# Hfx-J/SGTD

Measured on AMD Instinct MI355X. Metric: query frames/sec vs map size (descriptor build + candidate selection), higher is better.
Workload: dtype f64

## Files before the change

include/sgtd_accel.h:

```cpp
#ifndef SGTD_ACCEL_H
#define SGTD_ACCEL_H

#include <stddef.h>
#include <stdint.h>

#ifdef __cplusplus
extern "C" {
#endif

typedef enum sgtd_status {
  SGTD_OK = 0,
  SGTD_ERR_INVALID = -1,
  SGTD_ERR_NO_DEVICE = -2,
  SGTD_ERR_HIP = -3,
  SGTD_ERR_CAPACITY = -4,
  SGTD_ERR_FRAME_LIMIT = -5,
  SGTD_ERR_UNSUPPORTED = -6,
  SGTD_ERR_STATE = -7,
  SGTD_ERR_IO = -8
} sgtd_status;

typedef struct sgtd_config {
  int32_t descriptor_near_num;
  int32_t candidate_num;
  int32_t max_frame_n;
  int32_t device_id;
  double descriptor_min_len;
  double descriptor_max_len;
  double std_side_resolution;
  double rough_dis_threshold;
  uint32_t first_frame_id;
  uint32_t reserved;
} sgtd_config;

typedef struct sgtd_desc_soa {
  double *side;
  double *angle;
  double *center;
  float *vertex;
  int32_t *label;
  uint32_t *frame;
  int32_t *node_id;
} sgtd_desc_soa;

typedef struct sgtd_stats {
  int64_t n_entries;
  int64_t n_buckets;
  int64_t n_frames;
  int64_t last_queries;
  int64_t last_D;
  int64_t last_P;
  int64_t last_M;
  int64_t last_cand_pairs;
  int64_t hbm_bytes_table;
  float ms_build, ms_sort, ms_probe, ms_votes, ms_topk, ms_count, ms_scan, ms_write, ms_total;
  int32_t overflowed;
  int32_t select_form;
  int64_t last_P_swept;
  double bucket_len_sq_over_E;
  int64_t tail_entries;
  float ms_finalize;
  float reserved2;
  int64_t batches_total;
  int64_t overflow_launches_total;
  int64_t reruns_total;
  int64_t rewrites_total;
  int64_t list_moves_total;
  int64_t last_list_moves;
  int64_t device_allocs_total;
  float ms_consistency_pairs, ms_consistency_greedy;
  int32_t consistency_rounds;
  int32_t reserved3;
} sgtd_stats;

typedef struct sgtd_engine *sgtd_handle;

void sgtd_default_config(sgtd_config *cfg);
int sgtd_create(const sgtd_config *cfg, sgtd_handle *out);
int sgtd_create_multi(const sgtd_config *cfg, const int *device_ids, int n_dev, sgtd_handle *out);
int sgtd_device_count(sgtd_handle h);
sgtd_handle sgtd_device_handle(sgtd_handle h, int k);
int sgtd_destroy(sgtd_handle h);
const char *sgtd_strerror(int status);
const char *sgtd_last_error(sgtd_handle h);

int sgtd_set_stream(sgtd_handle h, void *hip_stream);
int sgtd_set_timing(sgtd_handle h, int enabled);

uint32_t sgtd_label_code(int a, int b, int c);
uint64_t sgtd_table_key(uint32_t code, uint32_t x, uint32_t y, uint32_t z);
uint64_t sgtd_dedup_key(uint64_t mx, uint64_t my, uint64_t mz);

int sgtd_current_frame_id(sgtd_handle h, uint32_t *out);

int64_t sgtd_max_descs(sgtd_handle h, int n_keypoints);
int sgtd_build(sgtd_handle h, const float *xyz, const uint32_t *label, int n,
               sgtd_desc_soa *out, int64_t capacity, int64_t *n_out);

int sgtd_add(sgtd_handle h, const sgtd_desc_soa *d, int64_t n);

int sgtd_add_frames(sgtd_handle h, const float *xyz, const uint32_t *label,
                    const int64_t *kp_off, int n_frames, int device_ptrs);

int sgtd_finalize(sgtd_handle h);

int sgtd_remove_frames(sgtd_handle h, const uint32_t *frame_ids, int64_t n, int64_t *n_removed);

int sgtd_set_frame_filter(sgtd_handle h, uint32_t frame_lo, uint32_t n_frames, const uint64_t *rows, int n_rows);

int sgtd_set_frame_poses(sgtd_handle h, const uint32_t *frame_ids, const float *pose12, int64_t n);

int sgtd_set_position_prior(sgtd_handle h, const double *center, const double *radius, int n_rows, int dims);

int sgtd_attach_table(sgtd_handle view, sgtd_handle owner);

int sgtd_query_frames(sgtd_handle h, const float *xyz, const uint32_t *label,
                      const int64_t *kp_off, int n_queries, int device_ptrs);

int sgtd_loop_frames(sgtd_handle h, const float *xyz, const uint32_t *label, const int64_t *kp_off,
                     int n_frames, int32_t skip_near, int device_ptrs);

int sgtd_query_descs(sgtd_handle h, const sgtd_desc_soa *q, int64_t nq);

int sgtd_result_candidates(sgtd_handle h, int32_t *n_cand, int32_t *cand_frame,
                           int32_t *cand_votes, int64_t *pair_off);
int sgtd_export_candidates_dev(sgtd_handle h, int32_t *d_cand_frame, int32_t *d_cand_votes);
int64_t sgtd_candidate_export_ints(int n_queries, int cand_num);
int sgtd_set_candidate_export(sgtd_handle h, int32_t *d_packed, int64_t capacity_ints);
int sgtd_export_wait(sgtd_handle h, void *side_stream);
int sgtd_export_release(sgtd_handle h, void *side_stream);
int sgtd_merge_candidates_dev(sgtd_handle h, void *stream, const int32_t *d_gathered, int n_tables, int my_table, int n_queries,
                              int32_t *d_frame, int32_t *d_votes, int32_t *d_n_cand, int32_t *d_src, uint64_t *d_keep,
                              int32_t *d_flags);
int sgtd_gather_verified_dev(sgtd_handle h, void *stream, const double *d_gathered, int n_tables, const int32_t *d_src,
                             int n_queries, double *d_score, double *d_pose);
int sgtd_set_deferred_lists(sgtd_handle h, int on);
int sgtd_finish_lists(sgtd_handle h, const uint64_t *d_keep);
int sgtd_verify_masked(sgtd_handle h, const uint64_t *d_keep);

int sgtd_result_query_desc_count(sgtd_handle h, int q, int64_t *n);
int sgtd_result_pairs(sgtd_handle h, int q, int32_t *q_idx, int64_t *db_entry,
                      int64_t capacity, int64_t *n_pairs);
int sgtd_result_query_descs(sgtd_handle h, int q, sgtd_desc_soa *out,
                            int64_t capacity, int64_t *n_out);
int sgtd_result_votes(sgtd_handle h, int q, uint32_t *votes, int64_t capacity,
                      uint32_t *frame_lo, int64_t *n);
int sgtd_result_rough(sgtd_handle h, int q, int32_t *q_idx, int32_t *cell,
                      int64_t *db_entry, uint32_t *frame, double *dis,
                      int64_t capacity, int64_t *n_rough);

int sgtd_verify(sgtd_handle h);
int sgtd_result_verify(sgtd_handle h, int q, double *score, double *pose);
int sgtd_result_world_poses(sgtd_handle h, int q, float *world);

int sgtd_refine_poses(sgtd_handle h, int iterations);
int sgtd_result_refined(sgtd_handle h, int q,
                        double *pose,
                        double *rmse,
                        double *rmse_verify,
                        int32_t *n_pairs,
                        double *moments);
int sgtd_result_refined_world_poses(sgtd_handle h, int q, float *world);

int sgtd_set_frame_keypoints(sgtd_handle h, const uint32_t *frame_ids, const int64_t *kp_off,
                             const float *xyz, const uint32_t *label, int64_t n);

#define SGTD_OVERLAP_REFINED 1
int sgtd_overlap(sgtd_handle h, double radius, int flags,
                 const float *q_xyz, const uint32_t *q_label, const int64_t *q_kp_off);
int sgtd_result_overlap(sgtd_handle h, int q,
                        int32_t *n_query_kp,
                        int32_t *n_frame_kp,
                        int32_t *n_hit_query,
                        int32_t *n_hit_frame,
                        double *overlap,
                        double *rms);
int sgtd_search_loop_overlap(sgtd_handle h, double icp_threshold, double min_overlap,
                             int32_t *best_cand, int32_t *best_frame,
                             double *best_score, double *best_overlap);

#define SGTD_ALIGN_REFINED 1
int sgtd_align_keypoints(sgtd_handle h, double radius, int iterations, int flags,
                         const float *q_xyz, const uint32_t *q_label, const int64_t *q_kp_off);
int sgtd_result_aligned(sgtd_handle h, int q,
                        double *pose,
                        int32_t *n_fits,
                        int32_t *n_corr,
                        int32_t *stop,
                        int32_t *counts_before,
                        int32_t *counts_after,
                        double *overlap_before,
                        double *rms_before,
                        double *overlap_after,
                        double *rms_after,
                        double *moments);
int sgtd_result_aligned_pairs(sgtd_handle h, int q, int cand, int32_t *frame_kp, int64_t capacity, int64_t *n);
int sgtd_result_aligned_world_poses(sgtd_handle h, int q, float *world);
int sgtd_search_loop_aligned(sgtd_handle h, double min_overlap, double max_rms,
                             int32_t *best_cand, int32_t *best_frame, double *best_rms, double *best_overlap);
int sgtd_export_verify_dev(sgtd_handle h, double *d_score, double *d_pose);
int sgtd_result_inliers(sgtd_handle h, int q, int cand, int32_t *idx, int64_t capacity, int64_t *n);
int sgtd_result_inlier_pairs(sgtd_handle h, int q, int64_t *cand_off, int32_t *q_idx, int64_t *db_entry,
                             int64_t capacity, int64_t *n_pairs);
int sgtd_result_inlier_entries(sgtd_handle h, int q, int64_t *cand_off, int32_t *q_idx, sgtd_desc_soa *entries,
                               int64_t capacity, int64_t *n_pairs);
int sgtd_search_loop(sgtd_handle h, double icp_threshold, int32_t *best_cand, int32_t *best_frame,
                     double *best_score);

#define SGTD_MAX_LOOP_EDGES 32768
int sgtd_consistent_loops(sgtd_handle h, int64_t n,
                          const uint32_t *frame_a,
                          const uint32_t *frame_b,
                          const double *rel_pose,
                          const float *pose_a,
                          double max_trans, double max_rot , int32_t *n_set);
int sgtd_result_consistent(sgtd_handle h, int32_t *in_set , int32_t *degree ,
                           int32_t *pick , double *thresholds );
int sgtd_result_consistency_rows(sgtd_handle h, int64_t first, int64_t n_rows, uint64_t *rows);
#define SGTD_LOOP_EDGES_REFINED 1
int sgtd_result_loop_edges(sgtd_handle h, double icp_threshold, int flags,
                           int32_t *query, uint32_t *frame_a, uint32_t *frame_b, double *rel_pose, double *score,
                           int64_t capacity, int64_t *n_edges);

#define SGTD_CONSENSUS_REFINED 1
#define SGTD_CONSENSUS_ALIGNED 2
int sgtd_pose_consensus_rows(sgtd_handle h, int64_t n_queries, int cand_num,
// ... 91 lines not shown
```

sgtd_amd/_lib.py:

```python
import ctypes as C
import os
import subprocess

_HERE = os.path.dirname(os.path.abspath(__file__))
LIB_PATH = os.environ.get("SGTD_ACCEL_LIB") or os.path.join(_HERE, "libsgtd_accel.so")
CSRC = os.path.join(_HERE, "csrc")

SGTD_OK = 0
ERRORS = {-8: "IO", -1: "INVALID", -2: "NO_DEVICE", -3: "HIP", -4: "CAPACITY",
          -5: "FRAME_LIMIT", -6: "UNSUPPORTED", -7: "STATE"}

SYMBOLS = [
    "sgtd_default_config", "sgtd_create", "sgtd_create_multi", "sgtd_device_count", "sgtd_device_handle", "sgtd_destroy", "sgtd_strerror", "sgtd_last_error", "sgtd_label_code", "sgtd_table_key", "sgtd_dedup_key",
    "sgtd_set_stream", "sgtd_set_timing", "sgtd_current_frame_id", "sgtd_max_descs", "sgtd_build",
    "sgtd_add", "sgtd_add_frames", "sgtd_finalize", "sgtd_query_frames", "sgtd_query_descs", "sgtd_max_batch",
    "sgtd_result_candidates", "sgtd_export_candidates_dev", "sgtd_result_query_desc_count", "sgtd_result_pairs",
    "sgtd_result_query_descs", "sgtd_result_votes", "sgtd_result_rough", "sgtd_fetch_entries", "sgtd_host_alloc", "sgtd_host_free",
    "sgtd_table_dump", "sgtd_sync", "sgtd_get_stats",
    "sgtd_verify", "sgtd_export_verify_dev", "sgtd_result_verify", "sgtd_result_inliers", "sgtd_result_inlier_pairs", "sgtd_result_inlier_entries", "sgtd_search_loop",
    "sgtd_graphs_load", "sgtd_graphs_save_cache", "sgtd_graphs_load_cache", "sgtd_graphs_view",
    "sgtd_graphs_error", "sgtd_graphs_free", "sgtd_save_table", "sgtd_load_table",
    "sgtd_candidate_export_ints", "sgtd_set_candidate_export", "sgtd_export_wait", "sgtd_export_release", "sgtd_merge_candidates_dev",
    "sgtd_gather_verified_dev", "sgtd_set_deferred_lists", "sgtd_finish_lists", "sgtd_verify_masked", "sgtd_attach_table", "sgtd_search_frame",
    "sgtd_loop_frames", "sgtd_remove_frames", "sgtd_set_frame_filter",
    "sgtd_set_frame_poses", "sgtd_set_position_prior", "sgtd_result_world_poses",
    "sgtd_refine_poses", "sgtd_result_refined", "sgtd_result_refined_world_poses",
    "sgtd_set_frame_keypoints", "sgtd_overlap", "sgtd_result_overlap", "sgtd_search_loop_overlap",
    "sgtd_align_keypoints", "sgtd_result_aligned", "sgtd_result_aligned_pairs", "sgtd_result_aligned_world_poses",
    "sgtd_search_loop_aligned",
    "sgtd_consistent_loops", "sgtd_result_consistent", "sgtd_result_consistency_rows", "sgtd_result_loop_edges",
    "sgtd_default_relax_options", "sgtd_relax_poses", "sgtd_result_relaxed",
    "sgtd_pose_consensus_rows", "sgtd_pose_consensus", "sgtd_result_consensus", "sgtd_result_consensus_rows",
    "sgtd_search_loop_consensus", "sgtd_result_consensus_edges",
]


class SgtdError(RuntimeError):
    def __init__(self, status, detail=""):
        self.status = status
        super().__init__("sgtd_accel: %s (%d) %s" % (ERRORS.get(status, "?"), status, detail))


class Config(C.Structure):
    _fields_ = [
        ("descriptor_near_num", C.c_int32),
        ("candidate_num", C.c_int32),
        ("max_frame_n", C.c_int32),
        ("device_id", C.c_int32),
        ("descriptor_min_len", C.c_double),
        ("descriptor_max_len", C.c_double),
        ("std_side_resolution", C.c_double),
        ("rough_dis_threshold", C.c_double),
        ("first_frame_id", C.c_uint32),
        ("reserved", C.c_uint32),
    ]


class DescSoa(C.Structure):
    _fields_ = [("side", C.c_void_p), ("angle", C.c_void_p), ("center", C.c_void_p),
                ("vertex", C.c_void_p), ("label", C.c_void_p), ("frame", C.c_void_p),
                ("node_id", C.c_void_p)]


class FrameSearch(C.Structure):
    _fields_ = [("n_cand", C.c_int32), ("flags", C.c_int32), ("cand_frame", C.c_void_p), ("cand_votes", C.c_void_p),
                ("pair_off", C.c_void_p), ("score", C.c_void_p), ("pose", C.c_void_p), ("inlier_off", C.c_void_p),
                ("inlier_q_idx", C.c_void_p), ("entries", DescSoa), ("capacity", C.c_int64), ("n_inliers", C.c_int64)]


class Stats(C.Structure):
    _fields_ = [
        ("n_entries", C.c_int64), ("n_buckets", C.c_int64), ("n_frames", C.c_int64),
        ("last_queries", C.c_int64), ("last_D", C.c_int64), ("last_P", C.c_int64),
        ("last_M", C.c_int64), ("last_cand_pairs", C.c_int64), ("hbm_bytes_table", C.c_int64),
        ("ms_build", C.c_float), ("ms_sort", C.c_float), ("ms_probe", C.c_float),
        ("ms_votes", C.c_float), ("ms_topk", C.c_float),
        ("ms_count", C.c_float), ("ms_scan", C.c_float), ("ms_write", C.c_float),
        ("ms_total", C.c_float), ("overflowed", C.c_int32), ("select_form", C.c_int32),
        ("last_P_swept", C.c_int64), ("bucket_len_sq_over_E", C.c_double),
        ("tail_entries", C.c_int64), ("ms_finalize", C.c_float), ("reserved2", C.c_float),
        ("batches_total", C.c_int64), ("overflow_launches_total", C.c_int64), ("reruns_total", C.c_int64), ("rewrites_total", C.c_int64),
        ("list_moves_total", C.c_int64), ("last_list_moves", C.c_int64), ("device_allocs_total", C.c_int64),
        ("ms_consistency_pairs", C.c_float), ("ms_consistency_greedy", C.c_float), ("consistency_rounds", C.c_int32), ("reserved3", C.c_int32),
    ]


class RelaxOptions(C.Structure):
    _fields_ = [("max_outer", C.c_int32), ("max_inner", C.c_int32), ("lambda_init", C.c_double), ("lambda_min", C.c_double),
                ("lambda_max", C.c_double), ("cg_tol", C.c_double), ("step_tol", C.c_double)]


class RelaxReport(C.Structure):
    _fields_ = [("cost_before", C.c_double), ("cost_after", C.c_double), ("lambda_", C.c_double),
                ("outer_iterations", C.c_int32), ("steps_accepted", C.c_int32), ("cg_iterations", C.c_int32), ("status", C.c_int32)]


def build_library(force=False):
    srcs = [os.path.join(CSRC, f) for f in os.listdir(CSRC)] + [
        os.path.join(os.path.dirname(_HERE), "include", "sgtd_accel.h")]
    stale = (not os.path.exists(LIB_PATH) or
             os.path.getmtime(LIB_PATH) < max(os.path.getmtime(s) for s in srcs))
    if force or stale:
        subprocess.check_call(["make", "-C", CSRC, "-s"] + (["-B"] if force else []))
    return LIB_PATH


_lib = None


def lib():
    global _lib
    if _lib is not None:
        return _lib
    if not os.path.exists(LIB_PATH):
        raise SgtdError(-2, "libsgtd_accel.so is not built (run __graft_entry__.build() or "
                            "make -C sgtd_amd/csrc); there is no CPU fallback")
    if os.environ.get("SGTD_NO_TORCH_PRELOAD") != "1":
        try:
            import torch
        except ImportError:
            pass
    L = C.CDLL(LIB_PATH)
    vp, i32, i64 = C.c_void_p, C.c_int32, C.c_int64
    L.sgtd_default_config.argtypes = [C.POINTER(Config)]
    L.sgtd_default_config.restype = None
    L.sgtd_create.argtypes = [C.POINTER(Config), C.POINTER(vp)]
    L.sgtd_destroy.argtypes = [vp]
    L.sgtd_create_multi.argtypes = [C.POINTER(Config), C.POINTER(C.c_int), C.c_int, C.POINTER(vp)]
    L.sgtd_device_count.argtypes = [vp]
    L.sgtd_device_handle.argtypes = [vp, C.c_int]
    L.sgtd_device_handle.restype = vp
    L.sgtd_strerror.argtypes = [C.c_int]
    L.sgtd_strerror.restype = C.c_char_p
    L.sgtd_last_error.argtypes = [vp]
    L.sgtd_last_error.restype = C.c_char_p
    L.sgtd_label_code.argtypes = [C.c_int] * 3
    L.sgtd_label_code.restype = C.c_uint32
    L.sgtd_table_key.argtypes = [C.c_uint32] * 4
    L.sgtd_table_key.restype = C.c_uint64
    L.sgtd_dedup_key.argtypes = [C.c_uint64] * 3
    L.sgtd_dedup_key.restype = C.c_uint64
    L.sgtd_set_stream.argtypes = [vp, vp]
    L.sgtd_set_timing.argtypes = [vp, C.c_int]
    L.sgtd_current_frame_id.argtypes = [vp, C.POINTER(C.c_uint32)]
    L.sgtd_max_descs.argtypes = [vp, C.c_int]
    L.sgtd_max_descs.restype = i64
    L.sgtd_build.argtypes = [vp, vp, vp, C.c_int, C.POINTER(DescSoa), i64, C.POINTER(i64)]
    L.sgtd_add.argtypes = [vp, C.POINTER(DescSoa), i64]
    L.sgtd_add_frames.argtypes = [vp, vp, vp, vp, C.c_int, C.c_int]
    L.sgtd_finalize.argtypes = [vp]
    L.sgtd_remove_frames.argtypes = [vp, vp, i64, C.POINTER(i64)]
    L.sgtd_set_frame_filter.argtypes = [vp, C.c_uint32, C.c_uint32, vp, C.c_int]
    L.sgtd_set_frame_poses.argtypes = [vp, vp, vp, i64]
    L.sgtd_set_position_prior.argtypes = [vp, vp, vp, C.c_int, C.c_int]
    L.sgtd_result_world_poses.argtypes = [vp, C.c_int, vp]
    L.sgtd_refine_poses.argtypes = [vp, C.c_int]
    L.sgtd_result_refined.argtypes = [vp, C.c_int, vp, vp, vp, vp, vp]
    L.sgtd_result_refined_world_poses.argtypes = [vp, C.c_int, vp]
    L.sgtd_set_frame_keypoints.argtypes = [vp, vp, vp, vp, vp, i64]
    L.sgtd_overlap.argtypes = [vp, C.c_double, C.c_int, vp, vp, vp]
    L.sgtd_result_overlap.argtypes = [vp, C.c_int, vp, vp, vp, vp, vp, vp]
    L.sgtd_search_loop_overlap.argtypes = [vp, C.c_double, C.c_double, vp, vp, vp, vp]
    L.sgtd_align_keypoints.argtypes = [vp, C.c_double, C.c_int, C.c_int, vp, vp, vp]
    L.sgtd_result_aligned.argtypes = [vp, C.c_int, vp, vp, vp, vp, vp, vp, vp, vp, vp, vp, vp]
    L.sgtd_result_aligned_pairs.argtypes = [vp, C.c_int, C.c_int, vp, i64, vp]
    L.sgtd_result_aligned_world_poses.argtypes = [vp, C.c_int, vp]
    L.sgtd_search_loop_aligned.argtypes = [vp, C.c_double, C.c_double, vp, vp, vp, vp]
    L.sgtd_consistent_loops.argtypes = [vp, i64, vp, vp, vp, vp, C.c_double, C.c_double, C.POINTER(i32)]
    L.sgtd_result_consistent.argtypes = [vp, vp, vp, vp, vp]
    L.sgtd_result_consistency_rows.argtypes = [vp, i64, i64, vp]
    L.sgtd_result_loop_edges.argtypes = [vp, C.c_double, C.c_int, vp, vp, vp, vp, vp, i64, C.POINTER(i64)]
    L.sgtd_default_relax_options.argtypes = [C.POINTER(RelaxOptions)]
    L.sgtd_default_relax_options.restype = None
    L.sgtd_relax_poses.argtypes = [vp, i64, vp, vp, i64, vp, vp, vp, vp, vp, C.POINTER(RelaxOptions), C.POINTER(RelaxReport)]
    L.sgtd_result_relaxed.argtypes = [vp, vp, vp]
    L.sgtd_pose_consensus_rows.argtypes = [vp, i64, C.c_int, vp, vp, vp, vp, C.c_double, C.c_double]
    L.sgtd_pose_consensus.argtypes = [vp, C.c_double, C.c_double, C.c_int]
    L.sgtd_result_consensus.argtypes = [vp, i64, i64, vp, vp, vp, vp, vp, vp, vp, vp, vp]
    L.sgtd_result_consensus_rows.argtypes = [vp, C.c_int, vp, vp, vp]
    L.sgtd_search_loop_consensus.argtypes = [vp, C.c_int, vp, vp, vp, vp]
    L.sgtd_result_consensus_edges.argtypes = [vp, C.c_int, vp, vp, vp, vp, vp, i64, C.POINTER(i64)]
    L.sgtd_query_frames.argtypes = [vp, vp, vp, vp, C.c_int, C.c_int]
    L.sgtd_loop_frames.argtypes = [vp, vp, vp, vp, C.c_int, i32, C.c_int]
    L.sgtd_query_descs.argtypes = [vp, C.POINTER(DescSoa), i64]
    L.sgtd_result_candidates.argtypes = [vp, vp, vp, vp, vp]
    L.sgtd_export_candidates_dev.argtypes = [vp, vp, vp]
    L.sgtd_result_query_desc_count.argtypes = [vp, C.c_int, C.POINTER(i64)]
    L.sgtd_result_pairs.argtypes = [vp, C.c_int, vp, vp, i64, C.POINTER(i64)]
    L.sgtd_result_query_descs.argtypes = [vp, C.c_int, C.POINTER(DescSoa), i64, C.POINTER(i64)]
    L.sgtd_result_votes.argtypes = [vp, C.c_int, vp, i64, C.POINTER(C.c_uint32), C.POINTER(i64)]
    L.sgtd_result_rough.argtypes = [vp, C.c_int, vp, vp, vp, vp, vp, i64, C.POINTER(i64)]
    L.sgtd_fetch_entries.argtypes = [vp, vp, i64, C.POINTER(DescSoa)]
    L.sgtd_table_dump.argtypes = [vp, vp, vp, vp, i64, i64]
    L.sgtd_sync.argtypes = [vp]
    L.sgtd_max_batch.argtypes = [vp, C.c_int, C.POINTER(C.c_int64)]
    L.sgtd_get_stats.argtypes = [vp, C.POINTER(Stats)]
    L.sgtd_verify.argtypes = [vp]
    L.sgtd_result_verify.argtypes = [vp, C.c_int, vp, vp]
    L.sgtd_export_verify_dev.argtypes = [vp, vp, vp]
    L.sgtd_result_inliers.argtypes = [vp, C.c_int, C.c_int, vp, i64, C.POINTER(i64)]
    L.sgtd_result_inlier_pairs.argtypes = [vp, C.c_int, vp, vp, vp, i64, C.POINTER(i64)]
    L.sgtd_result_inlier_entries.argtypes = [vp, C.c_int, vp, vp, C.POINTER(DescSoa), i64, C.POINTER(i64)]
    L.sgtd_host_alloc.argtypes = [C.c_size_t, C.POINTER(vp)]
    L.sgtd_host_free.argtypes = [vp]
    L.sgtd_search_loop.argtypes = [vp, C.c_double, vp, vp, vp]
    L.sgtd_graphs_load.argtypes = [C.POINTER(C.c_char_p), C.c_int, C.c_int, C.POINTER(vp)]
    L.sgtd_graphs_save_cache.argtypes = [vp, C.c_char_p]
    L.sgtd_graphs_load_cache.argtypes = [C.c_char_p, C.POINTER(vp)]
    L.sgtd_graphs_view.argtypes = [vp, C.POINTER(C.c_int), C.POINTER(i64), C.POINTER(vp), C.POINTER(vp),
                                   C.POINTER(vp), C.POINTER(vp)]
    L.sgtd_graphs_error.argtypes = [vp]
    L.sgtd_graphs_error.restype = C.c_char_p
    L.sgtd_graphs_free.argtypes = [vp]
    L.sgtd_graphs_free.restype = None
    L.sgtd_candidate_export_ints.argtypes = [C.c_int, C.c_int]
    L.sgtd_candidate_export_ints.restype = i64
    L.sgtd_set_candidate_export.argtypes = [vp, vp, i64]
    L.sgtd_export_wait.argtypes = [vp, vp]
    L.sgtd_export_release.argtypes = [vp, vp]
    L.sgtd_merge_candidates_dev.argtypes = [vp, vp, vp, C.c_int, C.c_int, C.c_int, vp, vp, vp, vp, vp, vp]
    L.sgtd_gather_verified_dev.argtypes = [vp, vp, vp, C.c_int, vp, C.c_int, vp, vp]
    L.sgtd_set_deferred_lists.argtypes = [vp, C.c_int]
    L.sgtd_finish_lists.argtypes = [vp, vp]
    L.sgtd_verify_masked.argtypes = [vp, vp]
    L.sgtd_attach_table.argtypes = [vp, vp]
    L.sgtd_search_frame.argtypes = [vp, C.POINTER(DescSoa), i64, C.POINTER(FrameSearch)]
    L.sgtd_save_table.argtypes = [vp, C.c_char_p]
    L.sgtd_load_table.argtypes = [vp, C.c_char_p]
    for name in SYMBOLS:
        getattr(L, name)
        if getattr(L, name).restype is C.c_int:
            pass
    _lib = L
    return L
```

sgtd_amd/csrc/multi_impl.hip.h:

```cpp
#pragma once
namespace multi {

static inline Group *G(sgtd_engine *e) { return e->grp; }

#define MCHK(call)                     \
  do {                                 \
    int _r = (call);                   \
    if (_r != SGTD_OK) {               \
      e->err = "device shard: " + std::string(sgtd_last_error(c)); \
      return _r;                       \
    }                                  \
  } while (0)

static void stale_stages(Group *g) { g->refined = false; g->overlapped = false; g->aligned = false; }
static void new_results(Group *g, bool verified) { g->verified = verified; stale_stages(g); }

template <class Call>
static int fan_out(sgtd_engine *e, const char *stage, const char *refined_flag, bool *done, Call call) {
  Group *g = G(e);
  if (!g->batch_valid || !g->verified) return needs(e, stage, "sgtd_verify");
  if (refined_flag && !g->refined) return needs(e, refined_flag, "sgtd_refine_poses");
  *done = false;
  for (sgtd_engine *c : g->dev) MCHK(call(c));
  *done = true;
// ... 503 lines not shown
  const double nan = std::numeric_limits<double>::quiet_NaN();
  struct Owned { std::vector<int32_t> c[4]; std::vector<double> ov, rms; };
  std::vector<Owned> own(g->n);
  int32_t *out[4] = {n_query_kp, n_frame_kp, n_hit_query, n_hit_frame};
  for (int k = 0; k < cn; k++) {
    for (int a = 0; a < 4; a++) if (out[a]) out[a][k] = -1;
    if (overlap) overlap[k] = nan;
    if (rms) rms[k] = nan;
  }
  return gather(e, q, [&](sgtd_engine *c, int s) {
    Owned &o = own[s];
    for (int a = 0; a < 4; a++) o.c[a].resize(cn);
    o.ov.resize(cn); o.rms.resize(cn);
    return sgtd_result_overlap(c, q, o.c[0].data(), o.c[1].data(), o.c[2].data(), o.c[3].data(), o.ov.data(), o.rms.data());
  }, [&](int s, int ks, int k) {
    const Owned &o = own[s];
    for (int a = 0; a < 4; a++) if (out[a]) out[a][k] = o.c[a][ks];
    if (overlap) overlap[k] = o.ov[ks];
    if (rms) rms[k] = o.rms[ks];
  });
}

int has_aligned(sgtd_engine *e) {
  Group *g = G(e);
  return g->batch_valid && g->verified && g->aligned;
}

int align_keypoints(sgtd_engine *e, double radius, int iterations, int flags, const float *q_xyz, const uint32_t *q_label, const int64_t *q_kp_off) {
  return fan_out(e, "sgtd_align_keypoints", (flags & SGTD_ALIGN_REFINED) ? "SGTD_ALIGN_REFINED" : nullptr, &G(e)->aligned,
                 [&](sgtd_engine *c) { return sgtd_align_keypoints(c, radius, iterations, flags, q_xyz, q_label, q_kp_off); });
}

int result_aligned(sgtd_engine *e, int q, double *pose, int32_t *n_fits, int32_t *n_corr, int32_t *stop, int32_t *counts_before, int32_t *counts_after,
                   double *overlap_before, double *rms_before, double *overlap_after, double *rms_after, double *moments) {
  Group *g = G(e);
  CHK(group_result_ready(e, q, g->aligned, kNoAligned));
  const int cn = e->cfg.candidate_num;
  const double nan = std::numeric_limits<double>::quiet_NaN();
  struct Owned { std::vector<double> pose, mom, val[4]; std::vector<int32_t> fit[3], cnt[2]; };
  std::vector<Owned> own(g->n);
  int32_t *fit[3] = {n_fits, n_corr, stop}, *cnt[2] = {counts_before, counts_after};
  double *val[4] = {overlap_before, rms_before, overlap_after, rms_after};
  for (int k = 0; k < cn; k++) {
    if (pose) std::fill(pose + (size_t)k * 12, pose + (size_t)k * 12 + 12, 0.0);
    if (moments) std::fill(moments + (size_t)k * 15, moments + (size_t)k * 15 + 15, nan);
    for (int a = 0; a < 3; a++) if (fit[a]) fit[a][k] = a == 2 ? -1 : 0;
    for (int a = 0; a < 2; a++) if (cnt[a]) std::fill(cnt[a] + (size_t)k * 4, cnt[a] + (size_t)k * 4 + 4, -1);
    for (int a = 0; a < 4; a++) if (val[a]) val[a][k] = nan;
  }
  return gather(e, q, [&](sgtd_engine *c, int s) {
    Owned &o = own[s];
    o.pose.resize((size_t)cn * 12); o.mom.resize((size_t)cn * 15);
    for (int a = 0; a < 4; a++) o.val[a].resize(cn);
    for (int a = 0; a < 3; a++) o.fit[a].resize(cn);
    for (int a = 0; a < 2; a++) o.cnt[a].resize((size_t)cn * 4);
    return sgtd_result_aligned(c, q, o.pose.data(), o.fit[0].data(), o.fit[1].data(), o.fit[2].data(), o.cnt[0].data(), o.cnt[1].data(),
                               o.val[0].data(), o.val[1].data(), o.val[2].data(), o.val[3].data(), o.mom.data());
  }, [&](int s, int ks, int k) {
    const Owned &o = own[s];
    if (pose) std::copy(o.pose.begin() + (size_t)ks * 12, o.pose.begin() + (size_t)ks * 12 + 12, pose + (size_t)k * 12);
    if (moments) std::copy(o.mom.begin() + (size_t)ks * 15, o.mom.begin() + (size_t)ks * 15 + 15, moments + (size_t)k * 15);
    for (int a = 0; a < 3; a++) if (fit[a]) fit[a][k] = o.fit[a][ks];
    for (int a = 0; a < 2; a++) if (cnt[a]) std::copy(o.cnt[a].begin() + (size_t)ks * 4, o.cnt[a].begin() + (size_t)ks * 4 + 4, cnt[a] + (size_t)k * 4);
    for (int a = 0; a < 4; a++) if (val[a]) val[a][k] = o.val[a][ks];
  });
}

int result_aligned_pairs(sgtd_engine *e, int q, int cand, int32_t *frame_kp, int64_t capacity, int64_t *n) {
  Group *g = G(e);
  CHK(group_result_ready(e, q, g->aligned, kNoAligned));
  if (cand < 0 || cand >= g->n_cand[q]) return SGTD_ERR_INVALID;
  const size_t i = (size_t)q * e->cfg.candidate_num + cand;
  sgtd_engine *c = g->dev[g->owner[i]];
  MCHK(sgtd_result_aligned_pairs(c, q, g->owner_slot[i], frame_kp, capacity, n));
  return SGTD_OK;
}

int result_inliers(sgtd_engine *e, int q, int cand, int32_t *idx, int64_t capacity, int64_t *n) {
  Group *g = G(e);
  if (!g->verified || q < 0 || q >= g->nq || cand < 0 || cand >= g->n_cand[q]) return SGTD_ERR_INVALID;
  const size_t i = (size_t)q * e->cfg.candidate_num + cand;
  sgtd_engine *c = g->dev[g->owner[i]];
  MCHK(sgtd_result_inliers(c, q, g->owner_slot[i], idx, capacity, n));
  return SGTD_OK;
}

int result_inlier_pairs(sgtd_engine *e, int q, int64_t *cand_off, int32_t *q_idx, int64_t *db_entry, int64_t capacity, int64_t *n_pairs) {
  Group *g = G(e);
  if (!n_pairs || !cand_off || !g->verified || q < 0 || q >= g->nq) return SGTD_ERR_INVALID;
  const int cn = e->cfg.candidate_num;
  std::vector<std::vector<int32_t>> qi(g->n);
  std::vector<std::vector<int64_t>> en(g->n), off(g->n);
  int64_t o = 0;
  bool fits = true;
  for (int k = 0; k <= cn; k++) cand_off[k] = 0;
  CHK(gather(e, q, [&](sgtd_engine *c, int s) {
    off[s].resize((size_t)cn + 1);
    int64_t ns = 0;
    const int st = sgtd_result_inlier_pairs(c, q, off[s].data(), nullptr, nullptr, 0, &ns);
    if (st != SGTD_OK && st != SGTD_ERR_CAPACITY) return st;
    qi[s].resize((size_t)std::max<int64_t>(ns, 1)); en[s].resize((size_t)std::max<int64_t>(ns, 1));
    return sgtd_result_inlier_pairs(c, q, off[s].data(), qi[s].data(), en[s].data(), ns, &ns);
  }, [&](int s, int ks, int k) {
    cand_off[k] = o;
    for (int64_t r = off[s][(size_t)ks]; r < off[s][(size_t)ks + 1]; r++, o++) {
      if (o < capacity) {
        if (q_idx) q_idx[o] = qi[s][(size_t)r];
        if (db_entry) db_entry[o] = ((int64_t)s << SGTD_ENTRY_SHARD_SHIFT) | en[s][(size_t)r];
      } else fits = false;
    }
  }));
  for (int k = g->n_cand[q]; k <= cn; k++) cand_off[k] = o;
  *n_pairs = o;
  return fits ? SGTD_OK : SGTD_ERR_CAPACITY;
}

int search_loop(sgtd_engine *e, double icp_threshold, int32_t *best_cand, int32_t *best_frame, double *best_score) {
  Group *g = G(e);
  if (!g->verified) return SGTD_ERR_INVALID;
  const int cn = e->cfg.candidate_num;
  std::vector<double> score(cn);
  for (int q = 0; q < g->nq; q++) {
    CHK(result_verify(e, q, score.data(), nullptr));
    double best = 0; int arg = -1;
    for (int k = 0; k < g->n_cand[q]; k++)
      if (score[k] > best) { best = score[k]; arg = k; }
    const bool ok = arg >= 0 && best > icp_threshold;
    if (best_cand) best_cand[q] = ok ? arg : -1;
    if (best_frame) best_frame[q] = ok ? g->cand_frame[(size_t)q * cn + arg] : -1;
    if (best_score) best_score[q] = ok ? best : 0.0;
  }
  return SGTD_OK;
}

int sync(sgtd_engine *e) {
  for (sgtd_engine *c : G(e)->dev) MCHK(sgtd_sync(c));
  return SGTD_OK;
}

int get_stats(sgtd_engine *e, sgtd_stats *out) {
  Group *g = G(e);
  sgtd_stats t{};
  for (int s = 0; s < g->n; s++) {
    sgtd_engine *c = g->dev[s];
    sgtd_stats x;
    MCHK(sgtd_get_stats(c, &x));
    t.n_entries += x.n_entries; t.n_buckets += x.n_buckets; t.n_frames += x.n_frames;
    t.last_queries = x.last_queries; t.last_D = x.last_D;
    t.last_P += x.last_P; t.last_M += x.last_M; t.last_P_swept += x.last_P_swept;
    t.hbm_bytes_table += x.hbm_bytes_table;
    t.overflowed |= x.overflowed;
    t.select_form = x.select_form;
    t.batches_total = x.batches_total; t.overflow_launches_total += x.overflow_launches_total;
    t.reruns_total += x.reruns_total; t.rewrites_total += x.rewrites_total;
    t.list_moves_total += x.list_moves_total; t.last_list_moves += x.last_list_moves;
    t.ms_total = std::max(t.ms_total, x.ms_total);
    if (s == 0) { t.ms_consistency_pairs = x.ms_consistency_pairs; t.ms_consistency_greedy = x.ms_consistency_greedy; t.consistency_rounds = x.consistency_rounds; }
  }
  if (g->merged) {
    const int cn = e->cfg.candidate_num;
    for (int q = 0; q < g->nq; q++) t.last_cand_pairs += g->pair_off[(size_t)q * (cn + 1) + cn];
  }
  *out = t;
  return SGTD_OK;
}

int max_batch(sgtd_engine *e, int n_keypoints, int64_t *max_queries) {
  int64_t best = -1;
  for (sgtd_engine *c : G(e)->dev) {
    int64_t m = 0;
    MCHK(sgtd_max_batch(c, n_keypoints, &m));
    best = best < 0 ? m : std::min(best, m);
  }
  *max_queries = best;
  return SGTD_OK;
}

u32 current_frame_id(sgtd_engine *e) { return G(e)->current_frame_id; }
int device_count(sgtd_engine *e) { return G(e)->n; }
sgtd_engine *device_handle(sgtd_engine *e, int k) { return (k >= 0 && k < G(e)->n) ? G(e)->dev[k] : nullptr; }

#undef MCHK
}
```

sgtd_amd/csrc/probe_kernels.hip.h:

```cpp
#pragma once
#include "common.hip.h"
#include <type_traits>

struct TableView {
  const HotEntry *ent;
  IdMap map;
  const double *cold_side;
  const BucketDir *dir;
  const HashSlot *hash;
  u32 hash_mask;
  u32 n_entries;
  u32 frame_lo;
  u32 frame_span;
  u32 coarse_at;
  u32 whole_at;
  u32 tail_off;
  const BucketDir *dir1;
  const HashSlot *hash1;
  u32 hash_mask1;
  u32 n_entries1;
};
__host__ __device__ __forceinline__ u32 group_row_bytes(const TableView &T) { return T.tail_off ? 2u * SGTD_GROUP_ROW_BYTES : SGTD_GROUP_ROW_BYTES; }

struct QueryView {
  const double *side;
  const QueryRec *qrec;
  const int *label;
  const u32 *frame;
  const u32 *count;
  long long stride;
  int n_queries;
  u32 chunk;
};

#define SGTD_REC_SHIFT 2
enum { CTR_REC_CURSOR = 0, CTR_AMB_COUNT = 2, CTR_COMPACT_CURSOR = 3, CTR_REC_NEED = 4, CTR_SWEPT = 6, CTR_POOL_CURSOR = 8, CTR_LIST_MOVES = 9,
       CTR_OVERFLOW = 10, CTR_COUNT = 12, CTR_XCD_HEADS = 1024 };
struct ProbeBuffers {
  u32 *rec;
  unsigned char *rec_cell;
  double *rec_dis;
  u32 rec_cap;
  u32 rec_slab;
  __host__ __device__ __forceinline__ size_t rec_index(u32 granule) const { return (size_t)granule << SGTD_REC_SHIFT; }
  __host__ __device__ __forceinline__ u32 *rec_at(u32 granule) const { return rec + ((size_t)granule << SGTD_REC_SHIFT); }
  u32 rec_rate;
  u32 *ctr;
  __host__ __device__ __forceinline__ unsigned long long *rec_cursor() const { return reinterpret_cast<unsigned long long *>(ctr + CTR_REC_CURSOR); }
  __host__ __device__ __forceinline__ u32 *amb_count() const { return ctr + CTR_AMB_COUNT; }
  __host__ __device__ __forceinline__ u32 *compact_cursor() const { return ctr + CTR_COMPACT_CURSOR; }
  __host__ __device__ __forceinline__ unsigned long long *rec_need() const { return reinterpret_cast<unsigned long long *>(ctr + CTR_REC_NEED); }
  __host__ __device__ __forceinline__ unsigned long long *swept() const { return reinterpret_cast<unsigned long long *>(ctr + CTR_SWEPT); }
  __host__ __device__ __forceinline__ u32 *pool_cursor() const { return ctr + CTR_POOL_CURSOR; }
  __host__ __device__ __forceinline__ u32 *list_moves() const { return ctr + CTR_LIST_MOVES; }
  __host__ __device__ __forceinline__ int *overflow() const { return reinterpret_cast<int *>(ctr + CTR_OVERFLOW); }
  __host__ __device__ __forceinline__ u32 *xcd_heads() const { return ctr + CTR_XCD_HEADS; }
  uint2 *list;
  u32 *n_visit;
  u32 *votes;
  u32 id_bits;
  uint2 *amb_queue;
  u32 amb_cap;
};

#define SGTD_PROBE_THREADS 256
#define SGTD_PROBE_CHUNK 128
#define SGTD_REC_SLAB 8192u
#define SGTD_SUB_DESCS 32
#ifndef SGTD_VOTE_WORDS
#define SGTD_VOTE_WORDS 6
#endif
#ifndef SGTD_WRITE_WORDS
#define SGTD_WRITE_WORDS 4
#endif

struct PendingLoads {
  u32 *h = nullptr, *a = nullptr, *b = nullptr, *c = nullptr;
  __device__ __forceinline__ void touch() const {
    if (a) asm volatile("" : "+v"(*h), "+v"(*a), "+v"(*b), "+v"(*c));
  }
};

#ifndef SGTD_PAIR
#define SGTD_PAIR 4
#endif
static_assert(SGTD_PAIR == 1 || SGTD_PAIR == 2 || SGTD_PAIR == 4, "the sweep computes the distances two at a time with packed f32 math");
#define SGTD_PASS_KMAX (SGTD_PAIR < 2 ? 2 : SGTD_PAIR)

struct WaveSlab {
  u32 state;
  u64 swept;
#ifdef SGTD_EXP_PHASE
  u64 ph[8], t;
#endif
};
#ifdef SGTD_EXP_PHASE
__device__ unsigned long long g_phase[8];
#define PH_ADD(i) do { const u64 _n = __builtin_readcyclecounter(); slab.ph[i] += _n - slab.t; slab.t = _n; } while (0)
#else
#define PH_ADD(i) do { } while (0)
#endif

__global__ __launch_bounds__(256) void query_prefix_kernel(const u32 *count, u32 *q_prefix, int n_queries,
                                                           u32 *n_valid) {
  __shared__ u32 lds[256 / SGTD_WAVE + 1];
  u32 carry = 0;
  for (int q0 = 0; q0 < n_queries; q0 += 256) {
    const int q = q0 + threadIdx.x;
    const u32 v = (q < n_queries) ? count[q] : 0;
    u32 tot;
    const u32 ex = block_excl_scan(v, lds, tot);
    if (q < n_queries) q_prefix[q] = carry + ex;
    carry += tot;
  }
  if (threadIdx.x == 0) *n_valid = carry;
}

__device__ __forceinline__ u64 home_coord(double s, u64 cmask) {
  return (int)(s - 1.0) < 0 ? cmask : min((u64)(u32)(int)s, cmask);
}

template <class KeyT>
__global__ void home_keys_kernel(QueryView Q, const u32 *q_prefix, KeyT *keys, u32 *vals, long long n_slots,
                                 int cbits, int sub_bits) {
  const long long d = (long long)blockIdx.x * blockDim.x + threadIdx.x;
  if (d >= n_slots) return;
  const int q = (int)(d / Q.stride);
  const u32 i = (u32)(d - (long long)q * Q.stride);
  if (i >= Q.count[q]) return;
  const u64 code = label_code(Q.label[d * 3 + 0], Q.label[d * 3 + 1], Q.label[d * 3 + 2]);
  const u64 cmask = (1ull << cbits) - 1ull;
  const u64 x = home_coord(Q.side[d * 3 + 0], cmask), y = home_coord(Q.side[d * 3 + 1], cmask),
            z = home_coord(Q.side[d * 3 + 2], cmask);
  const u32 idx = q_prefix[q] + i;
  const int ny = 1 << (sub_bits >> 1), nz = 1 << (sub_bits - (sub_bits >> 1));
  const double f1 = Q.side[d * 3 + 1] - (double)(int)Q.side[d * 3 + 1], f2 = Q.side[d * 3 + 2] - (double)(int)Q.side[d * 3 + 2];
  const u64 sub = (u64)min(max((int)(f1 * ny), 0), ny - 1) * nz + (u64)min(max((int)(f2 * nz), 0), nz - 1);
  keys[idx] = (KeyT)(((((code << cbits | x) << cbits | y) << cbits) | z) << sub_bits | sub);
  vals[idx] = (u32)d;
}

template <class KeyT>
__global__ void group_heads_kernel(const KeyT *keys, const u32 *n_valid_p, u32 *flags, long long n, int cbits, int sub_bits) {
  const long long p = (long long)blockIdx.x * blockDim.x + threadIdx.x;
  if (p >= n) return;
  u32 head = 0;
  if (p + 1 < (long long)*n_valid_p) {
    const u64 a = (u64)keys[p + 1] >> sub_bits, b = (u64)keys[p] >> sub_bits;
    const u64 cmask = (1ull << cbits) - 1ull;
    head = (a != b) || ((a & cmask) == cmask) || (((a >> cbits) & cmask) == cmask) ||
           (((a >> (2 * cbits)) & cmask) == cmask);
  }
  flags[p] = head;
}

__global__ void group_first_kernel(const u32 *gid, const u32 *n_valid_p, u32 *group_first, u32 *n_groups, long long n) {
  const long long p = (long long)blockIdx.x * blockDim.x + threadIdx.x;
  const long long nv = (long long)*n_valid_p;
  if (p >= n || p >= nv) return;
  const u32 g = gid[p];
  if (p == 0 || gid[p - 1] != g) group_first[g] = (u32)p;
  if (p == nv - 1) *n_groups = g + 1;
}

__global__ __launch_bounds__(256) void group_resolve_kernel(TableView T, QueryView Q, const u32 *order,
                                                            const u32 *group_first, const u32 *n_groups_p,
                                                            const u32 *n_valid_p, unsigned char *rows, u32 rows_cap,
                                                            int *overflow) {
  const int c = (int)(threadIdx.x & 31);
  const long long stride = ((long long)gridDim.x * blockDim.x) >> 5;
  const long long n_groups = (*n_valid_p) ? (long long)*n_groups_p : 0;
  if (n_groups > (long long)rows_cap) {
    if (blockIdx.x == 0 && threadIdx.x == 0) overflow[0] = 1;
    return;
  }
  for (long long g = ((long long)blockIdx.x * blockDim.x + threadIdx.x) >> 5; g < n_groups; g += stride) {
    if (c >= SGTD_NCELL) continue;
    const long long d = (long long)order[group_first[g]];
    const double q0 = Q.side[d * 3 + 0], q1 = Q.side[d * 3 + 1], q2 = Q.side[d * 3 + 2];
    const u32 code = label_code(Q.label[d * 3 + 0], Q.label[d * 3 + 1], Q.label[d * 3 + 2]);
    const int ix = c / 9 - 1, iy = (c / 3) % 3 - 1, iz = c % 3 - 1;
    const bool nonneg = q0 >= 0.0 && q1 >= 0.0 && q2 >= 0.0;
    const int x = nonneg ? max((int)q0 + ix, 0) : (int)(q0 + (double)ix);
    const int y = nonneg ? max((int)q1 + iy, 0) : (int)(q1 + (double)iy);
    const int z = nonneg ? max((int)q2 + iz, 0) : (int)(q2 + (double)iz);
    const bool minus_one = nonneg && ((ix < 0 && (int)(q0 + (double)ix) < 0) || (iy < 0 && (int)(q1 + (double)iy) < 0) ||
                                      (iz < 0 && (int)(q2 + (double)iz) < 0));
    const bool probe = !minus_one && x >= 0 && y >= 0 && z >= 0 && x < 65536 && y < 65536 && z < 65536;
    const u64 key = probe ? pack_key(code, (u32)x, (u32)y, (u32)z) : 0ull;
    for (int sg = 0; sg < (T.tail_off ? 2 : 1); sg++) {
// ... 1628 lines not shown
```

sgtd_amd/csrc/sgtd_accel.hip:

```cpp
#include "../../include/sgtd_accel.h"

#include <hip/hip_runtime.h>

#include <algorithm>
#include <atomic>
#include <chrono>
#include <cmath>
#include <cstdio>
#include <cstring>
#include <limits>
#include <memory>
#include <string>
#include <vector>

#include "build_kernel.hip.h"
#include "common.hip.h"
#include "table_kernels.hip.h"
#include "probe_kernels.hip.h"
#include "select_kernels.hip.h"
#include "verify_kernels.hip.h"
#include "verify_mfma.hip.h"
#include "exchange_kernels.hip.h"
#include "remove_kernels.hip.h"
#include "filter_kernels.hip.h"
#include "prior_kernels.hip.h"
#include "refine_kernels.hip.h"
#include "overlap_kernels.hip.h"
#include "align_kernels.hip.h"
#include "consistency_kernels.hip.h"
#include "relax_kernels.hip.h"
#include "consensus_kernels.hip.h"
#include "graph_ingest.hip.h"
#include "table_file.h"

namespace {

struct DevBuf {
  void *p = nullptr;
  size_t bytes = 0;
  bool borrowed = false;
  template <typename T> T *as() const { return reinterpret_cast<T *>(p); }
};

struct DescStore {
  DevBuf side, angle, center, vertex, label, frame, node_id, qrec;
  size_t cap = 0;
  bool with_thr2 = false;
  DescArrays view() const {
    DescArrays a;
    a.side = side.as<double>(); a.angle = angle.as<double>(); a.center = center.as<double>();
    a.vertex = vertex.as<float>(); a.label = label.as<int>(); a.frame = frame.as<u32>();
    a.node_id = node_id.as<int>();
    a.qrec = with_thr2 ? qrec.as<QueryRec>() : nullptr;
    return a;
  }
};

struct FrameFilter {
  u32 lo = 0, n = 0;
  int n_rows = 0;
  size_t words = 0;
  std::vector<u64> rows;
  u64 serial = 0;
  const u64 *row(int r) const { return rows.data() + (size_t)(n_rows == 1 ? 0 : r) * words; }
};

struct PositionPrior {
  int n_rows = 0, dims = 2;
  std::vector<double4> prm;
  u64 serial = 0;
};

static u64 row_bits_at(const u64 *row, size_t words, long long s) {
  const long long w = s >= 0 ? s / 64 : -((-s + 63) / 64);
  const int sh = (int)(s - w * 64);
  auto word = [&](long long i) -> u64 { return i >= 0 && i < (long long)words ? row[i] : 0ull; };
  return sh == 0 ? word(w) : (word(w) >> sh) | (word(w + 1) << (64 - sh));
}

template <class T>
struct PinnedVec {
  T *p = nullptr;
  size_t n = 0, cap = 0;
  PinnedVec() = default;
  PinnedVec(const PinnedVec &) = delete;
  PinnedVec &operator=(const PinnedVec &) = delete;
  ~PinnedVec() { if (p) (void)hipHostFree(p); }
  bool resize(size_t want) {
    if (want > cap) {
      void *np = nullptr;
      const size_t c = std::max<size_t>(want + want / 4, 64);
      if (hipHostMalloc(&np, c * sizeof(T), hipHostMallocDefault) != hipSuccess) return false;
      if (p) (void)hipHostFree(p);
      p = static_cast<T *>(np);
      cap = c;
    }
    n = want;
    return true;
  }
  T *data() { return p; }
  const T *data() const { return p; }
  T &operator[](size_t i) { return p[i]; }
  const T &operator[](size_t i) const { return p[i]; }
  size_t size() const { return n; }
};

constexpr size_t kCtrWords = CTR_XCD_HEADS + 8 * 1024;
enum { EV_START = 0, EV_BUILD, EV_SORT, EV_PROBE, EV_VOTES, EV_TOPK, EV_COUNT_T, EV_SCAN, EV_WRITE, EV_COUNT };

struct SelectPlan {
  int nq = 0, cn = 0; long long n_slots = 0; u32 span = 1, frame_lo = 0, id_bits = 13;
  u32 chunk = SGTD_PROBE_CHUNK; int blocks = 0, groups = 0, agrid = 0;
  u32 tile_span = 1, n_tiles = 1; size_t hist_bytes = 0; bool lds_votes = false;
  bool votes_fit = false, table_fits = false, per_query = false, fused_pairs = false, fused_votes = false, votes_per_query = false;
  int cbits = 1, sub_bits = 0, key_bits = 0; bool small = false, pair = false; size_t max_pass_slots = 0;
  int row_slots = 1; u32 ticket = 2; int sgrid = 0, pgrid = 0; bool narrow = false, frames = false;
  bool narrow_pairs = false;
};

}

namespace multi { struct Group; }

struct sgtd_engine {
  multi::Group *grp = nullptr;
  sgtd_config cfg;
  DevCfg dc;
  hipStream_t stream = nullptr;
  std::string err;
  int n_cus = 256;
  bool timing = false;
  hipEvent_t ev[EV_COUNT] = {};

  sgtd_engine *attached_to = nullptr;
  unsigned long long table_version = 0;
  unsigned long long attached_version = 0;
  int n_views = 0;
  u32 current_frame_id = 0;
  DescStore tab;
  int64_t n_entries = 0;
  int64_t n_add_calls = 0;
  bool have_frames = false;
  u32 frame_lo = 0, frame_hi = 0;
  bool finalized = false;

  struct Segment {
    DevBuf hot, perm, hash, bucket_start, bucket_key, dir;
    u32 hash_mask = 0;
    int64_t n_buckets = 0;
    int64_t g0 = 0, g1 = 0;
    double sum_len_sq = 0.0;
    u32 frame_hi = 0;
    bool built = false;
  };
  Segment seg[2];
  int n_seg = 1;
  u32 append_min_frame = 0xFFFFFFFFu;
  int64_t tail_max = 0;
  float ms_finalize = 0.f;
  u32 coarse_at = 62, whole_at = 62;
  long long thr2_pending = 0;
  u32 rec_rate_hook = 0;
  u32 rec_rate_cap = 256;
  bool wide_pairs = false;
  int tail_batches = 0;
  DevBuf slice_of, sq_sum;
  DevBuf frame_first, by_frame, id_of_g, longest;
  u32 id_bits = 0;
  bool id_by_frame = false;
  DevBuf rm_bits, rm_present, rm_mask, rm_count, rm_scratch;
  std::shared_ptr<const FrameFilter> filt, batch_filt;
  DevBuf filt_rows;
  std::vector<u64> filt_host;
  u64 filt_rows_serial = 0;
  u32 filt_rows_lo = 0, filt_rows_span = 0;
  std::vector<float> poses;
  std::vector<unsigned char> has_pose;
  u64 poses_serial = 0;
  std::shared_ptr<const PositionPrior> prior, batch_prior;
  DevBuf pos_dev, prior_dev, filt_base;
  std::vector<float4> pos_host;
  u64 pos_serial = 0;
  u32 pos_lo = 0, pos_span = 0;
  u64 filt_base_serial = 0;
  u32 filt_base_lo = 0, filt_base_span = 0;
  struct PriorKey {
    u64 prior = 0, poses = 0, filt = 0;
    u32 lo = 0, span = 0;
    int n_rows = 0;
    bool operator==(const PriorKey &o) const { return prior == o.prior && poses == o.poses && filt == o.filt && lo == o.lo && span == o.span && n_rows == o.n_rows; }
  } prior_key;
  bool prior_rows_valid = false;
  DevBuf keyA, keyB, valA, valB, hist, digit_tot, flags, bad_flag;
  std::vector<DevBuf> scan_lvl;

  DevBuf kp_off_dev, xyz_dev, label_dev, ws_keys, ws_slots, cnt_scan;
  DevBuf b_kp_off_dev, b_xyz_dev, b_label_dev;
  DescStore tmp;
  DescStore fetch;
  DevBuf fetch_idx;
  DevBuf tmp_count;

  DescStore qd;
  DevBuf q_count;
  long long q_stride = 0;
  int nq = 0;
  bool batch_valid = false, batch_synced = false;
  int last_kind = 0;
  const float *last_xyz = nullptr;
  const u32 *last_label = nullptr;
  std::vector<long long> last_kp_off;
  int last_max_n = 0;
  u32 last_qframe = 0;
  bool loop_batch = false;
  int loop_skip = 0;
  DevBuf totals;
  DevBuf cursors, list, n_visit, votes, slot_of;
  DevBuf q_M, q_P, q_pairs, q_pair_base, blk_count, rec, rec_cell, rec_dis;
  DevBuf c_pair, c_blk;
  DevBuf amb_queue;
  DevBuf n_cand, cand_frame, cand_votes, pair_off, pairs;
  DevBuf v_score, v_pose, v_inlier, v_best;
  DevBuf inl_pairs, inl_off;
  bool verify_counted = false;
  DevBuf inl_counts;
  DevBuf in_block;
  size_t frame_inl_cap = 0;
  char *frame_host = nullptr;
  size_t frame_host_bytes = 0;
  DevBuf b_in, b_out;
  char *pin_build = nullptr;
  size_t pin_build_cap = 0;
  DevBuf v_hyp64, v_hyp32, v_bound;
  DevBuf v_hypB, v_tau, v_words;
  DevBuf v_okey[2], v_oval[2];
  bool verified = false;
  DevBuf r_pose, r_rmse, r_rmse_v, r_npairs, r_moments, r_flag;
  bool refined = false;
  std::vector<std::vector<uint4>> kps;
  std::vector<unsigned char> has_kps;
  u64 kps_serial = 0, kp_dev_serial = 0;
  DevBuf kp_dev, kp_word, o_cnt, o_val, o_qxyz, o_qlabel, o_qoff;
  std::vector<uint4> kp_host;
  std::vector<u64> kp_word_host;
  int kp_dev_max = 0;
  bool overlapped = false;
  DevBuf a_pose, a_fit, a_cnt, a_val, a_mom, a_assign;
  std::vector<long long> a_qoff;
  bool aligned = false;
  DevBuf ck_store, ck_has, ck_in, ck_soa, ck_valid, ck_rows, ck_pmask, ck_out, ck_state;
  u64 ck_store_serial = ~0ull;
  int64_t ck_n = -1;
  double ck_thr[2] = {0.0, 0.0};
  hipEvent_t ck_ev[3] = {};
  DevBuf cs_in, cs_out;
  int64_t cs_n = -1;
  int cs_cn = 0;
  bool cs_batch = false;
  double cs_thr[2] = {0.0, 0.0};
  DevBuf rx_in, rx_state, rx_edge, rx_node, rx_ctl;
  int64_t rx_n = -1, rx_m = 0;
  int rx_cur = 0;
  int rx_max_blocks = 0;
  std::vector<int> rx_host_csr;
  std::vector<double> rx_host_w;
  std::vector<unsigned char> rx_host_held;
  int *export_packed = nullptr;
  size_t export_cap = 0;
  hipEvent_t ev_cand = nullptr, ev_export_free = nullptr;
  bool export_busy = false;
  u32 batch_serial = 0;
  bool defer_lists = false;
  bool lists_pending = false;
  bool lists_masked = false;
  const u64 *verify_keep = nullptr;
  const u64 *list_keep = nullptr;
  SelectPlan plan;
  DevBuf rough_qi, rough_entry, rough_frame, rough_cell, rough_dis;
  size_t rec_cap = (size_t)1 << 25;
  bool rec_cap_fixed = false;
  size_t pair_cap = (size_t)1 << 24;
  DevBuf n_valid, cell_rows, gid, q_prefix, group_first, n_groups;
  DevBuf pos_of_slot, rec_off, pass_pool;
  size_t pool_units = 0;
  size_t group_cap = 0;
  size_t group_cap_hook = 0;
  size_t amb_min = 65536;
  int sorted_chunk = 0;
  bool diag = false;
  int select_mode = 0;
  PinnedVec<u32> h_count, h_pair_base, h_q_M;
  PinnedVec<unsigned long long> h_q_P;
  PinnedVec<int> h_n_cand, h_cand_frame, h_cand_votes;
  PinnedVec<long long> h_pair_off;
  sgtd_stats stats{};
  char *pin = nullptr;
  size_t pin_cap = 0, pin_used = 0;
  struct PinCopy { void *dst; size_t off, bytes; };
  std::vector<PinCopy> pin_pending;
};

#include "multi.hip.h"

namespace {

#define HIPCHK(call)                                                          \
  do {                                                                        \
    hipError_t _s = (call);                                                   \
    if (_s != hipSuccess) {                                                   \
      e->err = std::string(#call) + ": " + hipGetErrorString(_s);             \
      return SGTD_ERR_HIP;                                                    \
    }                                                                         \
  } while (0)
#define CHK(call)                 \
  do {                            \
    int _r = (call);              \
    if (_r != SGTD_OK) return _r; \
  } while (0)

void stale_stages(sgtd_engine *e) {
  e->refined = false; e->overlapped = false; e->aligned = false;
  if (e->cs_batch) e->cs_n = -1;
}
void new_results(sgtd_engine *e, bool verified) { e->verified = verified; stale_stages(e); }

int ensure(sgtd_engine *e, DevBuf &b, size_t bytes, bool keep = false) {
  if (bytes <= b.bytes) return SGTD_OK;
  if (b.borrowed) { e->err = "a table attached from another handle cannot grow here"; return SGTD_ERR_STATE; }
  size_t want = keep ? std::max(bytes, b.bytes + b.bytes / 2) : (b.p ? bytes + bytes / 4 : bytes);
  if (!keep && b.p) {
    HIPCHK(hipStreamSynchronize(e->stream));
    HIPCHK(hipFree(b.p));
    b.p = nullptr; b.bytes = 0;
  }
  void *np = nullptr;
  {
    const hipError_t st_ = hipMalloc(&np, want);
    if (st_ != hipSuccess) {
      (void)hipGetLastError();
      e->err = "hipMalloc of " + std::to_string(want) + " bytes: " + hipGetErrorString(st_);
      return SGTD_ERR_HIP;
    }
  }
  e->stats.device_allocs_total++;
  if (keep && b.p && b.bytes) {
    HIPCHK(hipMemcpyAsync(np, b.p, b.bytes, hipMemcpyDeviceToDevice, e->stream));
    HIPCHK(hipStreamSynchronize(e->stream));
  }
  if (b.p) HIPCHK(hipFree(b.p));
  b.p = np;
  b.bytes = want;
  return SGTD_OK;
}

int ensure_store(sgtd_engine *e, DescStore &s, size_t cap, bool keep = false) {
  if (cap <= s.cap) return SGTD_OK;
  size_t want = keep ? std::max(cap, s.cap + s.cap / 2) : cap;
  CHK(ensure(e, s.side, want * 3 * sizeof(double), keep));
  CHK(ensure(e, s.angle, want * 3 * sizeof(double), keep));
  CHK(ensure(e, s.center, want * 3 * sizeof(double), keep));
  CHK(ensure(e, s.vertex, want * 9 * sizeof(float), keep));
  CHK(ensure(e, s.label, want * 3 * sizeof(int), keep));
  CHK(ensure(e, s.frame, want * sizeof(u32), keep));
  CHK(ensure(e, s.node_id, want * 3 * sizeof(int), keep));
  if (s.with_thr2) CHK(ensure(e, s.qrec, want * sizeof(QueryRec), keep));
  s.cap = want;
  return SGTD_OK;
}

void free_buf(DevBuf &b) {
  if (b.p && !b.borrowed) (void)hipFree(b.p);
  b.p = nullptr;
  b.bytes = 0;
  b.borrowed = false;
}
void free_store(DescStore &s) {
  free_buf(s.side); free_buf(s.angle); free_buf(s.center); free_buf(s.vertex);
  free_buf(s.label); free_buf(s.frame); free_buf(s.node_id); free_buf(s.qrec);
  s.cap = 0;
}

constexpr size_t kPinMax = (size_t)1 << 20, kPinCap = (size_t)16 << 20;

int xfer_sync(sgtd_engine *e) {
  HIPCHK(hipStreamSynchronize(e->stream));
  for (const auto &c : e->pin_pending) std::memcpy(c.dst, e->pin + c.off, c.bytes);
  e->pin_pending.clear();
  e->pin_used = 0;
  return SGTD_OK;
}

struct PinScope {
  sgtd_engine *e;
  explicit PinScope(sgtd_engine *e_) : e(e_) {}
  ~PinScope() {
    if (e && !e->pin_pending.empty()) {
      (void)hipStreamSynchronize(e->stream);
      e->pin_pending.clear();
      e->pin_used = 0;
    }
  }
};

int pin_room(sgtd_engine *e, size_t bytes, size_t *off) {
  if (!e->pin) {
    void *p = nullptr;
    HIPCHK(hipHostMalloc(&p, kPinCap, hipHostMallocDefault));
    e->pin = static_cast<char *>(p);
    e->pin_cap = kPinCap;
  }
  const size_t need = (bytes + 255) & ~(size_t)255;
  if (e->pin_used + need > e->pin_cap) CHK(xfer_sync(e));
  *off = e->pin_used;
  e->pin_used += need;
  return SGTD_OK;
}

int d2h(sgtd_engine *e, void *dst, const void *src_dev, size_t bytes) {
  if (bytes == 0) return SGTD_OK;
  if (bytes > kPinMax) {
    HIPCHK(hipMemcpyAsync(dst, src_dev, bytes, hipMemcpyDeviceToHost, e->stream));
    return SGTD_OK;
  }
  size_t off;
  CHK(pin_room(e, bytes, &off));
  HIPCHK(hipMemcpyAsync(e->pin + off, src_dev, bytes, hipMemcpyDeviceToHost, e->stream));
  e->pin_pending.push_back({dst, off, bytes});
  return SGTD_OK;
}

int h2d(sgtd_engine *e, void *dst_dev, const void *src, size_t bytes) {
  if (bytes == 0) return SGTD_OK;
  if (bytes > kPinMax) {
    HIPCHK(hipMemcpyAsync(dst_dev, src, bytes, hipMemcpyHostToDevice, e->stream));
    return SGTD_OK;
  }
  size_t off;
  CHK(pin_room(e, bytes, &off));
  std::memcpy(e->pin + off, src, bytes);
  HIPCHK(hipMemcpyAsync(dst_dev, e->pin + off, bytes, hipMemcpyHostToDevice, e->stream));
  return SGTD_OK;
}
// ... 328 lines not shown
  S.sum_len_sq = (double)sq;
  return SGTD_OK;
}

int build_idmap(sgtd_engine *e, u32 &bits) {
  const long long E = e->n_entries;
  bits = e->id_bits ? e->id_bits : 13;
  if (E == 0 || !e->have_frames) return SGTD_OK;
  const u32 lo = e->frame_lo, span = e->frame_hi - e->frame_lo + 1;
  const u32 *frame = e->tab.frame.as<u32>();
  CHK(ensure(e, e->frame_first, (size_t)span * sizeof(u32)));
  CHK(ensure(e, e->longest, 2 * sizeof(u32)));
  HIPCHK(hipMemsetAsync(e->longest.p, 0, 2 * sizeof(u32), e->stream));
  frame_monotone_kernel<<<grid_for(E, 256), 256, 0, e->stream>>>(frame, E, reinterpret_cast<int *>(e->longest.as<u32>() + 1));
  HIPCHK(hipGetLastError());
  u32 h[2] = {0, 0};
  HIPCHK(hipMemcpyAsync(h, e->longest.p, sizeof(h), hipMemcpyDeviceToHost, e->stream));
  HIPCHK(hipStreamSynchronize(e->stream));
  e->id_by_frame = h[1] != 0;
  const u32 *key = frame;
  if (e->id_by_frame) {
    CHK(ensure(e, e->keyA, (size_t)E * sizeof(u64)));
    CHK(ensure(e, e->keyB, (size_t)E * sizeof(u64)));
    CHK(ensure(e, e->valA, (size_t)E * sizeof(u32)));
    CHK(ensure(e, e->valB, (size_t)E * sizeof(u32)));
    u64 *kin = e->keyA.as<u64>(), *kout = e->keyB.as<u64>();
    u32 *vin = e->valA.as<u32>(), *vout = e->valB.as<u32>();
    frame_keys_kernel<<<grid_for(E, 256), 256, 0, e->stream>>>(frame, kin, vin, E);
    HIPCHK(hipGetLastError());
    CHK(radix_sort_pairs(e, kin, kout, vin, vout, E, 32, true));
    CHK(ensure(e, e->by_frame, (size_t)E * sizeof(u32)));
    CHK(ensure(e, e->id_of_g, (size_t)E * sizeof(u32)));
    HIPCHK(hipMemcpyAsync(e->by_frame.p, vin, (size_t)E * sizeof(u32), hipMemcpyDeviceToDevice, e->stream));
    low_words_kernel<<<grid_for(E, 256), 256, 0, e->stream>>>(kin, E, vout);
    HIPCHK(hipGetLastError());
    key = vout;
  }
  frame_first_kernel<<<grid_for(E, 256), 256, 0, e->stream>>>(key, E, lo, e->frame_first.as<u32>());
  HIPCHK(hipGetLastError());
  frame_longest_kernel<<<grid_for(E, 256), 256, 0, e->stream>>>(key, E, lo, e->frame_first.as<u32>(), e->longest.as<u32>());
  HIPCHK(hipGetLastError());
  HIPCHK(hipMemcpyAsync(h, e->longest.p, sizeof(u32), hipMemcpyDeviceToHost, e->stream));
  HIPCHK(hipStreamSynchronize(e->stream));
  u32 need = 1;
  while (need < 32 && (1ull << need) < (unsigned long long)h[0]) need++;
  auto fits = [&](u32 b) { return b < 32 && (unsigned long long)span < (1ull << (32 - b)) - 1ull; };
  if (bits < need || !fits(bits)) {
    bits = std::max<u32>(need, 13);
    if (!fits(bits)) bits = need;
    if (!fits(bits)) {
      e->err = "a 32-bit entry id cannot hold this table's frame span and its largest frame";
      return SGTD_ERR_UNSUPPORTED;
    }
  }
  if (e->id_by_frame) {
    id_of_sorted_kernel<<<grid_for(E, 256), 256, 0, e->stream>>>(key, e->by_frame.as<u32>(), E, lo, e->frame_first.as<u32>(), bits,
                                                                 e->id_of_g.as<u32>());
    HIPCHK(hipGetLastError());
  }
  return SGTD_OK;
}

int do_finalize(sgtd_engine *e, bool force_merge = false) {
  if (e->finalized && !(force_merge && e->n_seg > 1)) return SGTD_OK;
  if (e->attached_to) { e->err = "the table belongs to another handle (sgtd_attach_table): only its owner rebuilds it"; return SGTD_ERR_STATE; }
  e->table_version++;
  const long long E = e->n_entries;
  if (E >= (1ll << 32) - 2 - SGTD_SENTINELS) return SGTD_ERR_UNSUPPORTED;
  const auto t0 = std::chrono::steady_clock::now();
  sgtd_engine::Segment &M = e->seg[0], &T = e->seg[1];
  const long long tail_max = e->tail_max > 0 ? (long long)e->tail_max : std::max<long long>(262144, (M.g1 - M.g0) / 8);
  u32 bits = 0;
  CHK(build_idmap(e, bits));
  const bool can_tail = !force_merge && M.built && M.g0 == 0 && M.g1 > 0 && M.g1 <= E && E - M.g1 <= tail_max &&
                        bits == e->id_bits && !e->id_by_frame && (E == M.g1 || e->append_min_frame > M.frame_hi);
  e->id_bits = bits;
  if (can_tail) {
    if (E > M.g1) { CHK(build_segment(e, T, M.g1, E)); e->n_seg = 2; }
    else { T.built = false; e->n_seg = 1; }
  } else {
    CHK(build_segment(e, M, 0, E));
    T.built = false; T.g0 = T.g1 = E;
    e->n_seg = 1;
    e->append_min_frame = 0xFFFFFFFFu;
  }
  e->ms_finalize = std::chrono::duration<float, std::milli>(std::chrono::steady_clock::now() - t0).count();
  e->finalized = true;
  return SGTD_OK;
}

int rec_alloc(sgtd_engine *e, bool compact_lists) {
  CHK(ensure(e, e->rec, (e->rec_cap + 16) * sizeof(u32)));
  if (compact_lists) CHK(ensure(e, e->c_pair, std::min(e->rec_cap, kIndexLimit) * sizeof(u64)));
  if (e->diag) {
    CHK(ensure(e, e->rec_cell, e->rec_cap));
    CHK(ensure(e, e->rec_dis, e->rec_cap * sizeof(double)));
  }
  CHK(ensure(e, e->pairs, e->pair_cap * sizeof(u64)));
  CHK(ensure(e, e->amb_queue, std::max<size_t>(e->amb_min, e->rec_cap / 64) * sizeof(uint2)));
  return SGTD_OK;
}

constexpr double kDescsPerPass = SGTD_PAIR >= 4 ? 3.2 : (SGTD_PAIR >= 2 ? 1.9 : 1.0);
u32 pair_room(const sgtd_engine *e) { return (u32)std::min<size_t>(e->pair_cap, 0xFFFFFFF0u); }

struct Views {
  TableView T;
  QueryView Q;
  ProbeBuffers B;
  u32 span;
};

int launch_block_write(sgtd_engine *e, const SelectPlan &p, const Views &v, const CompactLists &CL) {
  auto write = [&](auto kernel) {
    kernel<<<p.agrid, 256, 0, e->stream>>>(v.Q, v.B, CL, p.blocks, e->blk_count.as<u32>(), p.cn, e->pair_off.as<long long>(), e->q_pair_base.as<u32>(),
                                           e->pairs.as<u64>(), v.T.map, e->n_cand.as<int>(), e->cand_frame.as<int>());
  };
  if (p.narrow_pairs) write(&block_write_kernel<true>); else write(&block_write_kernel<false>);
  HIPCHK(hipGetLastError());
  return SGTD_OK;
}

SelectPlan plan_select(const sgtd_engine *e) {
  SelectPlan p;
  const int nq = p.nq = e->nq, cn = p.cn = e->dc.cand_num;
  const long long n_slots = p.n_slots = (long long)nq * e->q_stride;
  const u32 span = p.span = e->have_frames ? (e->frame_hi - e->frame_lo + 1) : 1;
  p.frame_lo = e->have_frames ? e->frame_lo : 0;
  p.id_bits = e->id_bits ? e->id_bits : 13;
  while (p.chunk > SGTD_SUB_DESCS && (long long)nq * ((e->q_stride + p.chunk - 1) / p.chunk) < 1024) p.chunk >>= 1;
  if (const char *o = getenv("SGTD_BLOCK_CHUNK")) { const int c = atoi(o); if (c == 32 || c == 64 || c == 128) p.chunk = (u32)c; }
  p.blocks = (int)((e->q_stride + p.chunk - 1) / p.chunk);
  p.groups = (p.blocks + 3) / 4;
  p.agrid = ((nq + 7) / 8) * p.groups * 8;
  p.tile_span = span <= 36 * 1024 ? span : 36 * 1024;
  p.n_tiles = (span + p.tile_span - 1) / p.tile_span;
  p.hist_bytes = (size_t)span * sizeof(u32);
  p.lds_votes = p.hist_bytes <= 150 * 1024;
  static const size_t votes_room = lds_room(&votes_topk_kernel), list_room = lds_room(&pairs_query_kernel<true>);
  p.votes_fit = votes_topk_lds_bytes(span) <= votes_room;
  p.table_fits = (size_t)SGTD_PQ_TILE_RECS * sizeof(u32) + (((size_t)span + 15) & ~(size_t)15) + 16 <= list_room;
  p.per_query = e->select_mode == 2 || (e->select_mode == 0 && nq >= e->n_cus && (p.votes_fit || p.table_fits));
  p.fused_pairs = p.per_query && !e->wide_pairs && p.id_bits <= SGTD_PQ_RANK_BITS && !(cn == SGTD_MAX_CAND && p.id_bits == SGTD_PQ_RANK_BITS);
  p.fused_votes = p.fused_pairs && p.votes_fit;
  p.votes_per_query = p.n_tiles == 1 ? nq >= e->n_cus : ((long long)nq * p.n_tiles >= e->n_cus / 4 && p.n_tiles <= 8);
  p.narrow_pairs = p.id_bits <= SGTD_NARROW_RANK_BITS && !e->wide_pairs;
  while ((1ll << p.cbits) < (long long)(e->dc.max_len * e->dc.scale) + 3 && p.cbits < 16) p.cbits++;
  const int spare = (8 - (12 + 3 * p.cbits) % 8) % 8;
  p.sub_bits = spare >= 2 ? std::min(spare, 6) : 4;
  if (const char *o = getenv("SGTD_HOME_SUB_BITS")) p.sub_bits = std::min(6, std::max(0, atoi(o)));
  p.key_bits = 12 + 3 * p.cbits + p.sub_bits;
  const bool small_on = [] { const char *o = getenv("SGTD_SMALL_ORDER"); return !(o && !atoi(o)); }();
  p.small = small_on && nq == 1 && n_slots <= SGTD_SMALL_SLOTS && p.key_bits <= 32 && !p.fused_votes && span <= (1u << 20);
  p.pair = !e->diag && SGTD_PAIR >= 2;
  p.max_pass_slots = (size_t)pass_slot_count((u32)n_slots, (u32)n_slots, p.pair) + 64;
  p.row_slots = e->n_seg > 1 ? 2 : 1;
  if (e->stats.last_D > 0 && e->stats.last_P_swept > 0) {
    const double per_pass = (double)e->stats.last_P_swept / ((double)e->stats.last_D / (p.pair ? kDescsPerPass : 1.0));
    p.ticket = (u32)std::min(8.0, std::max(1.0, std::floor(1536.0 / per_pass + 0.5)));
  }
  if (e->sorted_chunk > 0) p.ticket = (u32)std::min(SGTD_TICKET_MAX, e->sorted_chunk);
  p.sgrid = e->n_cus * 8;
  if (const char *o = getenv("SGTD_SWEEP_BLOCKS_PER_CU")) p.sgrid = e->n_cus * std::max(1, atoi(o));
  int plan_per_cu = 20;
  if (const char *o = getenv("SGTD_PLAN_BLOCKS_PER_CU")) plan_per_cu = std::max(1, atoi(o));
  p.pgrid = (int)std::min<long long>(grid_for((long long)p.max_pass_slots, SGTD_PLAN_THREADS), (long long)e->n_cus * plan_per_cu);
  const u32 n0 = (u32)(e->seg[0].g1 - e->seg[0].g0), n1 = (u32)(e->seg[1].g1 - e->seg[1].g0);
  p.narrow = ((unsigned long long)n0 + SGTD_SENTINELS + (e->n_seg > 1 ? n1 + SGTD_SENTINELS : 0u)) * sizeof(HotEntry) < (1ull << 32);
  p.frames = e->last_kind != 1 || (e->have_frames && e->last_qframe >= e->frame_lo && e->last_qframe <= e->frame_hi);
  return p;
}

Views make_views(sgtd_engine *e) {
  const SelectPlan &p = e->plan;
  Views v;
  v.span = p.span;
  TableView &T = v.T;
  const sgtd_engine::Segment &S = e->seg[0], &S1 = e->seg[1];
  T.ent = S.hot.as<HotEntry>(); T.map = id_map(e, p.id_bits); T.cold_side = e->tab.side.as<double>();
  T.dir = S.dir.as<BucketDir>();
  T.hash = S.hash.as<HashSlot>(); T.hash_mask = S.hash_mask;
  T.coarse_at = e->coarse_at; T.whole_at = e->whole_at;
  T.n_entries = (u32)(S.g1 - S.g0); T.frame_lo = p.frame_lo; T.frame_span = v.span;
  T.tail_off = e->n_seg > 1 ? T.n_entries + SGTD_SENTINELS : 0u;
  T.dir1 = S1.dir.as<BucketDir>(); T.hash1 = S1.hash.as<HashSlot>(); T.hash_mask1 = S1.hash_mask;
  T.n_entries1 = e->n_seg > 1 ? (u32)(S1.g1 - S1.g0) : 0u;
  QueryView &Q = v.Q;
  Q.side = e->qd.side.as<double>(); Q.qrec = e->qd.qrec.as<QueryRec>();
  Q.label = e->qd.label.as<int>(); Q.frame = e->qd.frame.as<u32>();
  Q.count = e->q_count.as<u32>(); Q.stride = e->q_stride; Q.n_queries = e->nq; Q.chunk = p.chunk;
  ProbeBuffers &B = v.B;
  B.rec_cell = e->rec_cell.as<unsigned char>(); B.rec_dis = e->rec_dis.as<double>();
  B.rec_cap = (u32)std::min<size_t>(e->rec_cap >> SGTD_REC_SHIFT, kIndexLimit);
  B.rec = e->rec.as<u32>(); B.id_bits = p.id_bits;
  B.ctr = e->cursors.as<u32>();
  {
    const size_t streams = (size_t)e->n_cus * 32 * SGTD_PAIR;
    u32 slab = SGTD_REC_SLAB;
    while (slab > 512u && (size_t)slab * streams * 4 > e->rec_cap) slab >>= 1;
    if (const char *o = getenv("SGTD_REC_SLAB")) slab = (u32)std::max(512, atoi(o));
    B.rec_slab = slab >> SGTD_REC_SHIFT;
  }
  {
    const double per_pass = kDescsPerPass;
    B.rec_rate = 64;
    if (e->stats.last_P_swept > 0 && e->stats.last_M > 0) {
      const double meas = 256.0 * (double)e->stats.last_M / ((double)e->stats.last_P_swept * per_pass);
      const double scale = e->stats.last_queries > 0 ? (double)e->nq / (double)e->stats.last_queries : 1.0;
      const double fit = 256.0 * (0.6 * (double)e->rec_cap - 256.0 * (double)e->stats.last_D * scale) /
                         std::max(1.0, (double)e->stats.last_P_swept * scale * per_pass);
      const double want = std::max(std::min(3.0 * meas, fit), 1.2 * meas);
      B.rec_rate = (u32)std::min(256.0, std::max(want < 16.0 && fit < 16.0 ? 2.0 : 16.0, std::ceil(want)));
    }
    B.rec_rate = std::min(B.rec_rate, e->rec_rate_cap);
    if (e->diag) B.rec_rate = 256;
    if (e->rec_rate_hook) B.rec_rate = e->rec_rate_hook;
  }
  B.amb_queue = e->amb_queue.as<uint2>();
  B.amb_cap = (u32)std::min<size_t>(e->amb_queue.bytes / sizeof(uint2), 0xFFFFFFF0u);
  B.list = e->list.as<uint2>(); B.n_visit = e->n_visit.as<u32>();
  B.votes = e->votes.as<u32>();
  return v;
}

int launch_pairs_query(sgtd_engine *e, const Views &v, const u64 *keep = nullptr) {
  const int cn = e->dc.cand_num;
  const size_t img = (size_t)SGTD_PQ_TILE_RECS * sizeof(u32);
  const size_t tab = (((size_t)v.span + 15) & ~(size_t)15) + 16;
  const bool table = e->plan.table_fits;
  if (table) HIPCHK(hipFuncSetAttribute(reinterpret_cast<const void *>(&pairs_query_kernel<true>), hipFuncAttributeMaxDynamicSharedMemorySize, (int)(img + tab)));
  auto lists = [&](auto kernel) {
    kernel<<<e->nq, SGTD_PQ_THREADS, table ? img + tab : img, e->stream>>>(v.Q, v.B, e->n_cand.as<int>(), e->cand_frame.as<int>(), cn, e->pair_off.as<long long>(),
                                                                           e->q_pair_base.as<u32>(), e->pairs.as<u64>(), v.T.map, v.span, v.T.frame_lo, keep);
  };
  if (table) lists(&pairs_query_kernel<true>); else lists(&pairs_query_kernel<false>);
  HIPCHK(hipGetLastError());
  return SGTD_OK;
}

int export_candidates(sgtd_engine *e, const Views &v) {
  if (!e->export_packed) return SGTD_OK;
  const int nq = e->nq, cn = e->dc.cand_num;
  if (xchg_packed_ints(nq, cn) > e->export_cap) {
    e->err = "the registered candidate-export buffer is too small for this batch";
    return SGTD_ERR_CAPACITY;
  }
  if (e->export_busy) {
    HIPCHK(hipStreamWaitEvent(e->stream, e->ev_export_free, 0));
    e->export_busy = false;
  }
  export_candidates_kernel<<<std::min(grid_for((long long)nq * cn, 256), 512), 256, 0, e->stream>>>(
      e->cand_frame.as<int>(), e->cand_votes.as<int>(), v.B.overflow(), nq, cn, ++e->batch_serial, e->export_packed);
  HIPCHK(hipGetLastError());
  HIPCHK(hipEventRecord(e->ev_cand, e->stream));
  return SGTD_OK;
}

int launch_lists(sgtd_engine *e, const Views &v, const u64 *keep, bool first) {
  const int nq = e->nq, cn = e->dc.cand_num;
  if (keep) {
    cand_prefix_masked_kernel<<<grid_for(nq, 256), 256, 0, e->stream>>>(e->n_cand.as<int>(), e->cand_votes.as<int>(), keep, cn, nq,
                                                                          e->pair_off.as<long long>(), e->q_pairs.as<u32>());
    HIPCHK(hipGetLastError());
  } else if (!e->plan.fused_votes || e->lists_masked) {
    cand_prefix_kernel<<<grid_for(nq, 256), 256, 0, e->stream>>>(e->n_cand.as<int>(), e->cand_votes.as<int>(), cn, nq,
                                                                   e->pair_off.as<long long>(), e->q_pairs.as<u32>());
    HIPCHK(hipGetLastError());
  }
  e->lists_masked = keep != nullptr;
  e->list_keep = keep;
  if (e->timing && first) HIPCHK(hipEventRecord(e->ev[EV_COUNT_T], e->stream));
  if (!first) HIPCHK(hipMemsetAsync(v.B.overflow() + 1, 0, sizeof(int), e->stream));
  query_base_kernel<<<1, 256, 0, e->stream>>>(e->q_pairs.as<u32>(), e->q_pair_base.as<u32>(), nq, pair_room(e), v.B.overflow());
  HIPCHK(hipGetLastError());
  if (e->timing && first) HIPCHK(hipEventRecord(e->ev[EV_SCAN], e->stream));
  CHK(launch_pairs_query(e, v, keep));
  if (e->timing && first) HIPCHK(hipEventRecord(e->ev[EV_WRITE], e->stream));
  if (first) {
    batch_totals_kernel<<<1, 1, 0, e->stream>>>(v.B.ctr, e->totals.as<unsigned long long>());
    HIPCHK(hipGetLastError());
  }
  e->lists_pending = false;
  new_results(e, false);
  e->batch_synced = false;
  return SGTD_OK;
}

int rebase_filter(sgtd_engine *e, u32 frame_lo, u32 span, int n_rows, DevBuf &dst) {
  const FrameFilter &F = *e->batch_filt;
  const size_t words = ((size_t)span + 63) / 64;
  e->filt_host.assign((size_t)n_rows * words, 0ull);
  const long long shift = (long long)frame_lo - (long long)F.lo;
  const u64 last = span % 64 ? (1ull << (span % 64)) - 1ull : ~0ull;
  for (int r = 0; r < n_rows; r++) {
    u64 *dst = e->filt_host.data() + (size_t)r * words;
    for (size_t w = 0; w < words; w++) dst[w] = row_bits_at(F.row(r), F.words, shift + (long long)w * 64);
    dst[words - 1] &= last;
  }
  CHK(ensure(e, dst, e->filt_host.size() * sizeof(u64)));
  CHK(h2d(e, dst.p, e->filt_host.data(), e->filt_host.size() * sizeof(u64)));
  return SGTD_OK;
}

int prepare_filter(sgtd_engine *e, u32 frame_lo, u32 span) {
  const FrameFilter &F = *e->batch_filt;
  if (e->filt_rows.p && F.serial == e->filt_rows_serial && frame_lo == e->filt_rows_lo && span == e->filt_rows_span) return SGTD_OK;
  CHK(rebase_filter(e, frame_lo, span, F.n_rows == 1 ? 1 : e->nq, e->filt_rows));
  e->filt_rows_serial = F.serial; e->filt_rows_lo = frame_lo; e->filt_rows_span = span;
  e->prior_rows_valid = false;
  return SGTD_OK;
}

static int batch_row_count(const sgtd_engine *e) {
  const bool per_q = (e->batch_filt && e->batch_filt->n_rows > 1) || (e->batch_prior && e->batch_prior->n_rows > 1);
  return per_q ? e->nq : 1;
}

int prepare_prior(sgtd_engine *e, u32 frame_lo, u32 span) {
  const PositionPrior &P = *e->batch_prior;
  const int n_rows = batch_row_count(e);
  const sgtd_engine::PriorKey key{P.serial, e->poses_serial, e->batch_filt ? e->batch_filt->serial : 0ull, frame_lo, span, n_rows};
  if (e->filt_rows.p && e->prior_rows_valid && key == e->prior_key) return SGTD_OK;
  if (!e->pos_dev.p || e->pos_serial != e->poses_serial || e->pos_lo != frame_lo || e->pos_span != span) {
    e->pos_host.assign(span, make_float4(0.f, 0.f, 0.f, 0.f));
    const size_t n_ids = e->has_pose.size();
    for (u32 f = 0; f < span; f++) {
      const size_t id = (size_t)frame_lo + f;
      if (id >= n_ids) break;
      if (e->has_pose[id]) {
        const float *m = e->poses.data() + id * 12;
        e->pos_host[f] = make_float4(m[3], m[7], m[11], 1.f);
      }
    }
    CHK(ensure(e, e->pos_dev, (size_t)span * sizeof(float4)));
    CHK(h2d(e, e->pos_dev.p, e->pos_host.data(), (size_t)span * sizeof(float4)));
    e->pos_serial = e->poses_serial; e->pos_lo = frame_lo; e->pos_span = span;
  }
  CHK(ensure(e, e->prior_dev, P.prm.size() * sizeof(double4)));
  CHK(h2d(e, e->prior_dev.p, P.prm.data(), P.prm.size() * sizeof(double4)));
  const u64 *base = nullptr;
  int base_rows = 1;
  if (e->batch_filt) {
    const FrameFilter &F = *e->batch_filt;
    base_rows = F.n_rows == 1 ? 1 : e->nq;
    if (!e->filt_base.p || F.serial != e->filt_base_serial || frame_lo != e->filt_base_lo || span != e->filt_base_span) {
      CHK(rebase_filter(e, frame_lo, span, base_rows, e->filt_base));
      e->filt_base_serial = F.serial; e->filt_base_lo = frame_lo; e->filt_base_span = span;
    }
    base = e->filt_base.as<u64>();
  }
  const u32 words = (span + 63) / 64;
  CHK(ensure(e, e->filt_rows, (size_t)n_rows * words * sizeof(u64)));
  const long long waves = (long long)n_rows * words;
  const int grid = (int)((waves + SGTD_PRIOR_THREADS / SGTD_WAVE - 1) / (SGTD_PRIOR_THREADS / SGTD_WAVE));
  prior_rows_kernel<<<grid, SGTD_PRIOR_THREADS, 0, e->stream>>>(e->pos_dev.as<float4>(), span, words, e->prior_dev.as<double4>(),
                                                               P.n_rows == 1 ? 1 : n_rows, P.dims, base, base_rows, n_rows, e->filt_rows.as<u64>());
  HIPCHK(hipGetLastError());
  e->prior_key = key; e->prior_rows_valid = true;
  e->filt_rows_serial = 0;
  return SGTD_OK;
}

int launch_filter(sgtd_engine *e, const Views &v) {
  const int nq = e->nq, n_rows = batch_row_count(e);
  const u32 words = (v.span + 63) / 64;
  const long long chunks = (e->q_stride + SGTD_WAVE - 1) / SGTD_WAVE;
  const int want = (int)std::max<long long>(1, ((long long)e->n_cus * 8 + nq - 1) / nq);
  const int wg_per_q = (int)std::max<long long>(1, std::min<long long>(want, (chunks + SGTD_FILT_WAVES - 1) / SGTD_FILT_WAVES));
  const int grid = nq * wg_per_q;
  const size_t lds = (size_t)words * sizeof(u64);
  const u64 *rows = e->filt_rows.as<u64>();
  if (e->diag) {
    if (lds <= 65536) filter_compact_kernel<true><<<grid, SGTD_FILT_THREADS, lds, e->stream>>>(v.Q, v.B, rows, n_rows, words, v.span, wg_per_q);
    else filter_compact_kernel<false><<<grid, SGTD_FILT_THREADS, 0, e->stream>>>(v.Q, v.B, rows, n_rows, words, v.span, wg_per_q);
  } else {
    if (lds <= 65536)
      filter_records_kernel<true><<<grid, SGTD_FILT_THREADS, lds, e->stream>>>(v.Q, v.B, rows, n_rows, words, v.span, wg_per_q, e->q_M.as<u32>());
    else
      filter_records_kernel<false><<<grid, SGTD_FILT_THREADS, 0, e->stream>>>(v.Q, v.B, rows, n_rows, words, v.span, wg_per_q, e->q_M.as<u32>());
  }
  HIPCHK(hipGetLastError());
  return SGTD_OK;
}

int reserve_select(sgtd_engine *e, const SelectPlan &p) {
  const int nq = p.nq, cn = p.cn;
  const size_t slots = (size_t)std::max<long long>(p.n_slots, 1), n_slots = (size_t)p.n_slots;
  CHK(ensure(e, e->cursors, kCtrWords * sizeof(u32)));
  if (!e->totals.p) {
    CHK(ensure(e, e->totals, 4 * sizeof(unsigned long long)));
    HIPCHK(hipMemsetAsync(e->totals.p, 0, 4 * sizeof(unsigned long long), e->stream));
  }
  CHK(ensure(e, e->list, slots * sizeof(uint2)));
  CHK(ensure(e, e->n_visit, slots * sizeof(u32)));
  CHK(ensure(e, e->votes, (size_t)nq * p.span * sizeof(u32)));
  CHK(ensure(e, e->slot_of, (size_t)nq * p.span + 4));
  for (DevBuf *b : {&e->q_M, &e->q_pairs, &e->q_prefix}) CHK(ensure(e, *b, (size_t)nq * sizeof(u32)));
  CHK(ensure(e, e->q_P, (size_t)nq * sizeof(unsigned long long)));
  CHK(ensure(e, e->q_pair_base, (size_t)(nq + 1) * sizeof(u32)));
  CHK(ensure(e, e->blk_count, (size_t)nq * p.blocks * 64 * sizeof(u32)));
  CHK(ensure(e, e->c_blk, (size_t)nq * p.blocks * 2 * sizeof(u32)));
  CHK(ensure(e, e->n_cand, (size_t)nq * sizeof(int)));
  for (DevBuf *b : {&e->cand_frame, &e->cand_votes}) CHK(ensure(e, *b, (size_t)nq * cn * sizeof(int)));
  CHK(ensure(e, e->pair_off, (size_t)nq * (cn + 1) * sizeof(long long)));
  if (e->batch_prior) CHK(prepare_prior(e, p.frame_lo, p.span));
  else if (e->batch_filt) CHK(prepare_filter(e, p.frame_lo, p.span));
  CHK(rec_alloc(e, !p.fused_pairs));
  if (e->group_cap_hook) { if (e->group_cap == 0) e->group_cap = e->group_cap_hook; }
  else {
    const long long want = p.n_slots <= 65536 ? p.n_slots : std::min<long long>(p.n_slots / 2, std::max<long long>(p.n_slots / 8, 1500000));
    e->group_cap = std::max<size_t>(e->group_cap, (size_t)want);
  }
  CHK(ensure(e, e->cell_rows, std::max<size_t>(e->group_cap, 1) * SGTD_GROUP_ROW_BYTES * p.row_slots));
  for (DevBuf *b : {&e->keyA, &e->keyB}) CHK(ensure(e, *b, n_slots * sizeof(u64)));
  for (DevBuf *b : {&e->valA, &e->valB, &e->gid, &e->group_first}) CHK(ensure(e, *b, n_slots * sizeof(u32)));
  for (DevBuf *b : {&e->n_valid, &e->n_groups}) CHK(ensure(e, *b, sizeof(u32)));
  for (DevBuf *b : {&e->pos_of_slot, &e->rec_off}) CHK(ensure(e, *b, p.max_pass_slots * sizeof(u32)));
  if (e->pool_units == 0) e->pool_units = std::max<size_t>(65536, n_slots * (e->n_entries > 100000000 ? 16 : 10));
  CHK(ensure(e, e->pass_pool, (e->pool_units + SGTD_PASS_SLACK_UNITS) * sizeof(uint4)));
  return SGTD_OK;
}

int clear_batch(sgtd_engine *e, const SelectPlan &p) {
  const int nq = p.nq, cn = p.cn;
  if (e->thr2_pending > 0) {
    thr2_kernel<<<grid_for(e->thr2_pending, 256), 256, 0, e->stream>>>(e->qd.side.as<double>(), e->qd.frame.as<u32>(), e->qd.qrec.as<QueryRec>(), e->thr2_pending,
                                                                        e->dc.rough);
    HIPCHK(hipGetLastError());
  }
  if (p.small) return SGTD_OK;
  HIPCHK(hipMemsetAsync(e->cursors.p, 0, kCtrWords * sizeof(u32), e->stream));
  if (!p.fused_votes) {
    if (!p.votes_per_query) HIPCHK(hipMemsetAsync(e->votes.p, 0, (size_t)nq * p.span * sizeof(u32), e->stream));
    HIPCHK(hipMemsetAsync(e->slot_of.p, 0xFF, (size_t)nq * p.span, e->stream));
    HIPCHK(hipMemsetAsync(e->cand_frame.p, 0xFF, (size_t)nq * cn * sizeof(int), e->stream));
    HIPCHK(hipMemsetAsync(e->cand_votes.p, 0, (size_t)nq * cn * sizeof(int), e->stream));
  }
  HIPCHK(hipMemsetAsync(e->q_M.p, 0, (size_t)nq * sizeof(u32), e->stream));
  HIPCHK(hipMemsetAsync(e->q_P.p, 0, (size_t)nq * sizeof(unsigned long long), e->stream));
  return SGTD_OK;
}

int order_descriptors(sgtd_engine *e, const SelectPlan &p, const Views &v, u32 **order) {
  const long long n_slots = p.n_slots;
  u32 *vin = e->valA.as<u32>(), *vout = e->valB.as<u32>(), *gid = e->gid.as<u32>();
  const u32 *nv = e->n_valid.as<u32>();
  if (p.small) {
    SmallOrder SO;
    SO.ctr = e->cursors.as<u32>(); SO.ctr_words = (u32)kCtrWords;
    SO.q_M = e->q_M.as<u32>(); SO.q_P = e->q_P.as<unsigned long long>();
    SO.votes = p.votes_per_query ? nullptr : e->votes.as<u32>(); SO.slot_of_words = e->slot_of.as<u32>(); SO.span = p.span;
    SO.cand_frame = e->cand_frame.as<int>(); SO.cand_votes = e->cand_votes.as<int>(); SO.cand_num = p.cn;
    SO.q_prefix = e->q_prefix.as<u32>(); SO.n_valid = e->n_valid.as<u32>(); SO.order = vin; SO.gid = gid;
    SO.group_first = e->group_first.as<u32>(); SO.n_groups = e->n_groups.as<u32>(); SO.pos_of_slot = e->pos_of_slot.as<u32>();
    SO.n_slots = (u32)n_slots; SO.max_pass_slots = (u32)p.max_pass_slots; SO.cbits = p.cbits; SO.sub_bits = p.sub_bits; SO.pair = p.pair ? 1 : 0; SO.key_bits = p.key_bits;
    SO.qrec = nullptr; SO.n_qrec = 0; SO.rough = e->dc.rough;
    const size_t lds = (size_t)SGTD_SMALL_SLOTS * 16;
    HIPCHK(hipFuncSetAttribute(reinterpret_cast<const void *>(&small_order_kernel), hipFuncAttributeMaxDynamicSharedMemorySize, (int)lds));
    small_order_kernel<<<1, SGTD_SMALL_THREADS, lds, e->stream>>>(v.Q, SO);
    HIPCHK(hipGetLastError());
    e->thr2_pending = 0; *order = vin;
    return SGTD_OK;
  }
  query_prefix_kernel<<<1, 256, 0, e->stream>>>(e->q_count.as<u32>(), e->q_prefix.as<u32>(), p.nq, e->n_valid.as<u32>());
  HIPCHK(hipGetLastError());
  auto sort_by_home = [&](auto *kin, auto *kout) -> int {
    using Key = typename std::remove_pointer<decltype(kin)>::type;
    home_keys_kernel<Key><<<grid_for(n_slots, 256), 256, 0, e->stream>>>(v.Q, e->q_prefix.as<u32>(), kin, vin, n_slots, p.cbits, p.sub_bits);
    HIPCHK(hipGetLastError());
    CHK(radix_sort_pairs(e, kin, kout, vin, vout, n_slots, p.key_bits, false, nv));
    group_heads_kernel<Key><<<grid_for(n_slots, 256), 256, 0, e->stream>>>(kin, nv, gid, n_slots, p.cbits, p.sub_bits);
    HIPCHK(hipGetLastError());
    return SGTD_OK;
  };
  if (p.key_bits <= 32) CHK(sort_by_home(e->keyA.as<u32>(), e->keyB.as<u32>()));
  else CHK(sort_by_home(e->keyA.as<u64>(), e->keyB.as<u64>()));
  CHK(device_scan(e, gid, gid, n_slots));
  group_first_kernel<<<grid_for(n_slots, 256), 256, 0, e->stream>>>(gid, nv, e->group_first.as<u32>(), e->n_groups.as<u32>(), n_slots);
  HIPCHK(hipGetLastError());
  HIPCHK(hipMemsetAsync(e->pos_of_slot.p, 0xFF, p.max_pass_slots * sizeof(u32), e->stream));
  pass_slots_kernel<<<grid_for(n_slots, 256), 256, 0, e->stream>>>(gid, e->group_first.as<u32>(), nv, e->pos_of_slot.as<u32>(), n_slots, p.pair ? 1 : 0);
  HIPCHK(hipGetLastError());
  e->thr2_pending = 0; *order = vin;
  return SGTD_OK;
}

int plan_and_sweep(sgtd_engine *e, const SelectPlan &p, const Views &v, u32 *vin) {
  const u32 *nv = e->n_valid.as<u32>();
  const unsigned char *rows = e->cell_rows.as<unsigned char>();
  const u32 rows_cap = (u32)std::min<size_t>(e->group_cap, 0xFFFFFFFFu);
  PassPool PP;
  PP.pool = e->pass_pool.as<uint4>(); PP.rec_off = e->rec_off.as<u32>();
  PP.cursor = v.B.pool_cursor(); PP.cap = (u32)std::min<size_t>(e->pool_units, 0xFFFFFF00u);
  group_resolve_kernel<<<e->n_cus * 16, 256, 0, e->stream>>>(v.T, v.Q, vin, e->group_first.as<u32>(),
                                                              e->n_groups.as<u32>(), nv, e->cell_rows.as<unsigned char>(), rows_cap, v.B.overflow());
  HIPCHK(hipGetLastError());
#define SGTD_LAUNCH_PLAN(PR, TL)                                                                               \
  plan_passes_kernel<PR, TL><<<p.pgrid, SGTD_PLAN_THREADS, 0, e->stream>>>(v.T, v.Q, vin, e->gid.as<u32>(), e->pos_of_slot.as<u32>(), nv, \
                                                       e->n_groups.as<u32>(), rows, rows_cap, PP, v.B.n_visit, v.B.list,          \
                                                       v.B.overflow())
  if (v.T.tail_off) { if (p.pair) SGTD_LAUNCH_PLAN(true, true); else SGTD_LAUNCH_PLAN(false, true); }
  else { if (p.pair) SGTD_LAUNCH_PLAN(true, false); else SGTD_LAUNCH_PLAN(false, false); }
#undef SGTD_LAUNCH_PLAN
  HIPCHK(hipGetLastError());
  if (e->timing) HIPCHK(hipEventRecord(e->ev[EV_SORT], e->stream));
#define SGTD_LAUNCH_SORTED(DG, WD, FR, BD)                                                                      \
  probe_sorted_kernel<DG, WD, FR, BD><<<p.sgrid, SGTD_PROBE_THREADS, 0, e->stream>>>(                           \
      v.T, v.B, v.Q, PP, e->dc.rough, e->n_valid.as<u32>(), e->n_groups.as<u32>(), p.ticket)
  if (e->diag) {
    if (e->loop_batch) SGTD_LAUNCH_SORTED(true, true, true, true);
    else SGTD_LAUNCH_SORTED(true, true, true, false);
  } else if (e->loop_batch) {
    if (p.narrow) SGTD_LAUNCH_SORTED(false, false, true, true);
    else SGTD_LAUNCH_SORTED(false, true, true, true);
  }
  else if (p.narrow && p.frames) SGTD_LAUNCH_SORTED(false, false, true, false);
  else if (p.narrow) SGTD_LAUNCH_SORTED(false, false, false, false);
  else if (p.frames) SGTD_LAUNCH_SORTED(false, true, true, false);
  else SGTD_LAUNCH_SORTED(false, true, false, false);
#undef SGTD_LAUNCH_SORTED
  HIPCHK(hipGetLastError());
  resolve_undecided_kernel<<<64, 256, 0, e->stream>>>(v.T, v.Q, v.B, e->q_M.as<u32>());
  HIPCHK(hipGetLastError());
  if (e->batch_filt || e->batch_prior) CHK(launch_filter(e, v));
#ifdef SGTD_EXP_PHASE
  {
    static int pcalls = 0;
    if (++pcalls == 6) {
      HIPCHK(hipStreamSynchronize(e->stream));
      unsigned long long ph[8];
      HIPCHK(hipMemcpyFromSymbol(ph, HIP_SYMBOL(g_phase), sizeof(ph)));
      const double tot = (double)ph[7];
      fprintf(stderr, "PHASE (fractions of wave life, %llu waves): prologue %.3f locate+issue %.3f wait-loads %.3f test %.3f epilogue %.3f between-passes %.3f rest %.3f\n",
              ph[6], ph[0] / tot, ph[1] / tot, ph[2] / tot, ph[3] / tot, ph[4] / tot, ph[5] / tot,
              (tot - ph[0] - ph[1] - ph[2] - ph[3] - ph[4] - ph[5]) / tot);
    }
  }
#endif
  if (e->timing) HIPCHK(hipEventRecord(e->ev[EV_PROBE], e->stream));
  return SGTD_OK;
}

int launch_votes(sgtd_engine *e, const SelectPlan &p, const Views &v) {
  u32 *q_M = e->q_M.as<u32>();
  unsigned long long *q_P = e->q_P.as<unsigned long long>();
  if (p.fused_votes) {
    const size_t lds = votes_topk_lds_bytes(p.span);
    HIPCHK(hipFuncSetAttribute(reinterpret_cast<const void *>(&votes_topk_kernel), hipFuncAttributeMaxDynamicSharedMemorySize, (int)lds));
    votes_topk_kernel<<<p.nq, SGTD_VT_THREADS, lds, e->stream>>>(v.Q, v.B, p.span, v.T.frame_lo, p.blocks, p.cn, q_M, q_P, e->n_cand.as<int>(),
                                                                  e->cand_frame.as<int>(), e->cand_votes.as<int>(), e->pair_off.as<long long>(),
                                                                  e->q_pairs.as<u32>());
  } else if (p.votes_per_query) {
    const size_t tile_bytes = (size_t)p.tile_span * sizeof(u32);
    HIPCHK(hipFuncSetAttribute(reinterpret_cast<const void *>(&votes_query_kernel), hipFuncAttributeMaxDynamicSharedMemorySize, (int)tile_bytes));
    votes_query_kernel<<<p.nq * (int)p.n_tiles, SGTD_VOTES_Q_THREADS, tile_bytes, e->stream>>>(v.Q, v.B, p.span, v.T.frame_lo, p.tile_span, p.blocks, q_M, q_P);
  } else if (p.lds_votes) {
    HIPCHK(hipFuncSetAttribute(reinterpret_cast<const void *>(&votes_kernel<true>), hipFuncAttributeMaxDynamicSharedMemorySize, (int)p.hist_bytes));
    votes_kernel<true><<<p.agrid, 256, p.hist_bytes, e->stream>>>(v.Q, v.B, p.span, v.T.frame_lo, p.blocks, q_M, q_P);
  } else {
    votes_kernel<false><<<p.agrid, 256, 0, e->stream>>>(v.Q, v.B, p.span, v.T.frame_lo, p.blocks, q_M, q_P);
  }
  HIPCHK(hipGetLastError());
  if (e->timing) HIPCHK(hipEventRecord(e->ev[EV_VOTES], e->stream));
  return SGTD_OK;
}

int launch_topk(sgtd_engine *e, const SelectPlan &p, const Views &v) {
  if (!p.fused_votes) {
    topk_kernel<<<p.nq, SGTD_TOPK_THREADS, 0, e->stream>>>(e->votes.as<u32>(), p.span, v.T.frame_lo, p.cn, e->n_cand.as<int>(),
                                                            e->cand_frame.as<int>(), e->cand_votes.as<int>(), e->slot_of.as<unsigned char>());
    HIPCHK(hipGetLastError());
  }
  if (e->timing) HIPCHK(hipEventRecord(e->ev[EV_TOPK], e->stream));
  return SGTD_OK;
}

CompactLists compact_lists(sgtd_engine *e, const SelectPlan &p, const Views &v) {
  CompactLists CL;
  CL.pair = e->c_pair.as<u64>();
  CL.blk_start = e->c_blk.as<u32>(); CL.blk_n = e->c_blk.as<u32>() + (size_t)p.nq * p.blocks;
  CL.cursor = v.B.compact_cursor(); CL.cap = (u32)std::min<size_t>(e->c_pair.bytes / sizeof(u64), 0xFFFFFFF0u);
  return CL;
}

int launch_block_lists(sgtd_engine *e, const SelectPlan &p, const Views &v) {
  const int nq = p.nq;
  const CompactLists CL = compact_lists(e, p, v);
  const int sl_bytes = p.span <= 48 * 1024 ? (int)((p.span + 15) & ~15u) : 0;
  auto count = [&](auto kernel) -> int {
    if (sl_bytes) HIPCHK(hipFuncSetAttribute(reinterpret_cast<const void *>(kernel), hipFuncAttributeMaxDynamicSharedMemorySize, sl_bytes));
    kernel<<<p.agrid, 256, sl_bytes, e->stream>>>(v.Q, v.B, e->n_cand.as<int>(), e->cand_frame.as<int>(), p.cn, p.blocks, e->blk_count.as<u32>(), CL,
                                                  nullptr, nullptr, e->slot_of.as<unsigned char>(), p.span, v.T.frame_lo);
    HIPCHK(hipGetLastError());
    return SGTD_OK;
  };
  if (sl_bytes) CHK(p.narrow_pairs ? count(&block_count_kernel<true, true>) : count(&block_count_kernel<true, false>));
  else CHK(p.narrow_pairs ? count(&block_count_kernel<false, true>) : count(&block_count_kernel<false, false>));
  if (e->timing) HIPCHK(hipEventRecord(e->ev[EV_COUNT_T], e->stream));
  block_scan_kernel<<<nq, 64, 0, e->stream>>>(e->blk_count.as<u32>(), p.blocks, p.cn, e->n_cand.as<int>(),
                                               e->pair_off.as<long long>(), e->q_pairs.as<u32>(),
                                               v.B.overflow(), nq == 1 ? e->q_pair_base.as<u32>() : nullptr, pair_room(e),
                                               nq == 1 ? e->totals.as<unsigned long long>() : nullptr);
  HIPCHK(hipGetLastError());
  if (nq != 1) {
    query_base_kernel<<<1, 256, 0, e->stream>>>(e->q_pairs.as<u32>(), e->q_pair_base.as<u32>(), nq, pair_room(e), v.B.overflow());
    HIPCHK(hipGetLastError());
  }
  if (e->timing) HIPCHK(hipEventRecord(e->ev[EV_SCAN], e->stream));
  CHK(launch_block_write(e, p, v, CL));
  if (e->timing) HIPCHK(hipEventRecord(e->ev[EV_WRITE], e->stream));
  if (nq != 1) {
    batch_totals_kernel<<<1, 1, 0, e->stream>>>(v.B.ctr, e->totals.as<unsigned long long>());
    HIPCHK(hipGetLastError());
  }
  e->batch_valid = true;
  new_results(e, false);
  e->batch_synced = false;
  return SGTD_OK;
}

int launch_select(sgtd_engine *e) {
  e->plan = plan_select(e);
  const SelectPlan &p = e->plan;
  CHK(reserve_select(e, p));
  CHK(clear_batch(e, p));
  const Views v = make_views(e);
  u32 *order = nullptr;
  CHK(order_descriptors(e, p, v, &order));
  CHK(plan_and_sweep(e, p, v, order));
  CHK(launch_votes(e, p, v));
  CHK(launch_topk(e, p, v));
  CHK(export_candidates(e, v));
  e->lists_pending = false;
  e->lists_masked = false;
  e->stats.select_form = p.fused_votes ? 2 : (p.fused_pairs ? 1 : 0);
  if (!p.fused_pairs) return launch_block_lists(e, p, v);
  e->batch_valid = true;
  if (!e->defer_lists) return launch_lists(e, v, nullptr, true);
  if (e->timing)
    for (int k : {EV_COUNT_T, EV_SCAN, EV_WRITE}) HIPCHK(hipEventRecord(e->ev[k], e->stream));
  batch_totals_kernel<<<1, 1, 0, e->stream>>>(v.B.ctr, e->totals.as<unsigned long long>());
  HIPCHK(hipGetLastError());
  e->lists_pending = true;
  new_results(e, false);
  e->batch_synced = false;
  return SGTD_OK;
}

int enqueue_frames(sgtd_engine *e) {
  const int nq = e->nq;
  if (e->timing) HIPCHK(hipEventRecord(e->ev[EV_START], e->stream));
  CHK(launch_build(e, e->last_xyz, e->last_label, e->kp_off_dev.as<long long>(), nq, e->last_max_n,
                   e->last_qframe, e->loop_batch ? 1 : 0, e->qd.view(), e->q_stride, e->q_count.as<u32>()));
  if (e->loop_batch) {
    loop_bound_kernel<<<grid_for(e->q_stride * nq, 256), 256, 0, e->stream>>>(e->qd.qrec.as<QueryRec>(), e->q_stride, nq, e->last_qframe,
                                                                             e->loop_skip, e->have_frames ? e->frame_lo : 0);
    HIPCHK(hipGetLastError());
  }
  if (e->timing) HIPCHK(hipEventRecord(e->ev[EV_BUILD], e->stream));
  return launch_select(e);
}

int rerun(sgtd_engine *e) {
  if (e->last_kind == 1) return enqueue_frames(e);
  if (e->timing) HIPCHK(hipEventRecord(e->ev[EV_START], e->stream));
  return launch_select(e);
}

int rerun_write(sgtd_engine *e) {
  const SelectPlan &p = e->plan;
  CHK(ensure(e, e->pairs, e->pair_cap * sizeof(u64)));
  const Views v = make_views(e);
  HIPCHK(hipMemsetAsync(v.B.overflow() + 1, 0, sizeof(int), e->stream));
  if (p.fused_pairs) return launch_lists(e, v, e->lists_masked ? e->list_keep : nullptr, false);
  query_base_kernel<<<1, 256, 0, e->stream>>>(e->q_pairs.as<u32>(), e->q_pair_base.as<u32>(), p.nq, pair_room(e), v.B.overflow());
  HIPCHK(hipGetLastError());
  return launch_block_write(e, p, v, compact_lists(e, p, v));
}

int view_current(sgtd_engine *e) {
  if (!e->attached_to) return SGTD_OK;
  if (e->attached_to->table_version != e->attached_version || !e->attached_to->finalized) {
    e->err = "the owner's table changed since sgtd_attach_table: attach again";
    e->batch_valid = false;
    return SGTD_ERR_STATE;
  }
  return SGTD_OK;
}

void stage_times(sgtd_engine *e) {
  if (!e->timing) return;
  sgtd_stats &s = e->stats;
  auto el = [&](int a, int b) { float ms = 0; (void)hipEventElapsedTime(&ms, e->ev[a], e->ev[b]); return ms; };
  if (e->last_kind == 1) { s.ms_build = el(EV_START, EV_BUILD); s.ms_sort = el(EV_BUILD, EV_SORT); }
  else { s.ms_build = 0; s.ms_sort = el(EV_START, EV_SORT); }
  s.ms_probe = el(EV_SORT, EV_PROBE); s.ms_votes = el(EV_PROBE, EV_VOTES);
  s.ms_topk = el(EV_VOTES, EV_TOPK); s.ms_count = el(EV_TOPK, EV_COUNT_T);
  s.ms_scan = el(EV_COUNT_T, EV_SCAN); s.ms_write = el(EV_SCAN, EV_WRITE);
  s.ms_total = el(EV_START, EV_WRITE);
}

int sync_batch(sgtd_engine *e) {
  PinScope pin_scope(e);
  if (!e->batch_valid) return SGTD_ERR_STATE;
  CHK(view_current(e));
  if (e->batch_synced) return SGTD_OK;
  e->stats.overflowed = 0;
  unsigned long long swept = 0;
  for (int attempt = 0; attempt < 12; attempt++) {
    int ovf[2] = {0, 0};
    unsigned long long cursor = 0, need = 0;
    swept = 0;
    u32 total = 0, pool_used = 0;
    u32 ctr[CTR_COUNT];
    u32 n_groups = 0;
    unsigned long long tot[3] = {0, 0, 0};
    if (e->lists_pending) CHK(launch_lists(e, make_views(e), nullptr, false));
    CHK(d2h(e, ctr, e->cursors.p, sizeof(ctr)));
    if (e->totals.p) CHK(d2h(e, tot, e->totals.p, sizeof(tot)));
    if (e->n_groups.p) CHK(d2h(e, &n_groups, e->n_groups.p, sizeof(u32)));
    CHK(d2h(e, &total, e->q_pair_base.as<u32>() + e->nq, sizeof(u32)));
    CHK(xfer_sync(e));
    std::memcpy(&cursor, ctr + CTR_REC_CURSOR, 8); std::memcpy(&need, ctr + CTR_REC_NEED, 8); std::memcpy(&swept, ctr + CTR_SWEPT, 8);
    cursor <<= SGTD_REC_SHIFT;
    pool_used = ctr[CTR_POOL_CURSOR]; ovf[0] = (int)ctr[CTR_OVERFLOW]; ovf[1] = (int)ctr[CTR_OVERFLOW + 1];
    e->stats.last_list_moves = ctr[CTR_LIST_MOVES];
    e->stats.batches_total = (int64_t)tot[0]; e->stats.overflow_launches_total = (int64_t)tot[1]; e->stats.list_moves_total = (int64_t)tot[2];
    if (!ovf[0] && !ovf[1]) {
      const size_t lim0 = kRecLimit;
      if ((double)cursor * 1.1 > (double)e->rec_cap) e->rec_cap = std::min<size_t>(lim0, (size_t)((double)cursor * 1.5));
      break;
    }
    e->stats.overflowed = 1;
    if (ovf[0]) e->stats.reruns_total++; else e->stats.rewrites_total++;
    if (getenv("SGTD_DEBUG"))
      fprintf(stderr, "sgtd: batch re-run (attempt %d): flags %d %d, records %llu of %zu (+%llu wanted), pass pool %u of %zu units, home cells %u of %zu rows, pairs %u of %zu\n",
              attempt, ovf[0], ovf[1], cursor, e->rec_cap, need, pool_used, e->pool_units, n_groups, e->group_cap, total, e->pair_cap);
    if (attempt == 11) return SGTD_ERR_CAPACITY;
    const size_t lim = kRecLimit, pair_lim = kIndexLimit;
    if (ovf[0] && (size_t)n_groups > e->group_cap) {
      e->group_cap = (size_t)n_groups + (size_t)n_groups / 4 + 1024;
    } else if (ovf[0] && (size_t)pool_used > e->pool_units) {
      if (e->pool_units >= 0xFFFFFF00ull) return SGTD_ERR_CAPACITY;
      e->pool_units = std::min<size_t>(0xFFFFFF00ull, (size_t)pool_used + (size_t)pool_used / 4 + 65536);
    } else if (ovf[0]) {
      const bool reservations = (double)cursor > 1.5 * (double)e->rec_cap + 4.0 * (double)need;
      if (reservations && e->rec_rate_cap > 2) {
        e->rec_rate_cap = std::max<u32>(2, std::min<u32>(e->rec_rate_cap, 64) / 4);
      } else if (e->rec_cap >= lim) {
        return SGTD_ERR_CAPACITY;
      }
      const size_t want = (size_t)((double)(e->rec_cap + need) * 1.4) + (size_t)e->n_cus * 32 * SGTD_PAIR * 512;
      e->rec_cap = std::min<size_t>(lim, std::max<size_t>(reservations ? e->rec_cap : e->rec_cap * 2, want));
    } else if (ovf[1]) {
      if (e->pair_cap >= pair_lim) return SGTD_ERR_CAPACITY;
      e->pair_cap = std::min<size_t>(pair_lim, std::max<size_t>(e->pair_cap * 2, (size_t)total + (total >> 3) + 65536));
      CHK(rerun_write(e));
      continue;
    }
    CHK(rerun(e));
  }
  const int nq = e->nq, cn = e->dc.cand_num;
  if (!(e->h_count.resize(nq) && e->h_pair_base.resize(nq + 1) && e->h_q_M.resize(nq) && e->h_q_P.resize(nq) &&
        e->h_n_cand.resize(nq) && e->h_cand_frame.resize((size_t)nq * cn) && e->h_cand_votes.resize((size_t)nq * cn) &&
        e->h_pair_off.resize((size_t)nq * (cn + 1)))) {
    e->err = "hipHostMalloc of the result tables failed";
    return SGTD_ERR_HIP;
  }
  auto pull = [&](void *dst, const void *src, size_t bytes) { return bytes ? hipMemcpyAsync(dst, src, bytes, hipMemcpyDeviceToHost, e->stream) : hipSuccess; };
  HIPCHK(pull(e->h_count.data(), e->q_count.p, nq * sizeof(u32)));
  HIPCHK(pull(e->h_pair_base.data(), e->q_pair_base.p, (nq + 1) * sizeof(u32)));
  HIPCHK(pull(e->h_q_M.data(), e->q_M.p, nq * sizeof(u32)));
  HIPCHK(pull(e->h_q_P.data(), e->q_P.p, nq * sizeof(unsigned long long)));
  HIPCHK(pull(e->h_n_cand.data(), e->n_cand.p, nq * sizeof(int)));
  HIPCHK(pull(e->h_cand_frame.data(), e->cand_frame.p, (size_t)nq * cn * sizeof(int)));
  HIPCHK(pull(e->h_cand_votes.data(), e->cand_votes.p, (size_t)nq * cn * sizeof(int)));
  HIPCHK(pull(e->h_pair_off.data(), e->pair_off.p, (size_t)nq * (cn + 1) * sizeof(long long)));
  CHK(xfer_sync(e));
  sgtd_stats &s = e->stats;
  s.last_queries = nq;
  s.last_D = 0; s.last_P = 0; s.last_M = 0; s.last_cand_pairs = 0;
  s.last_P_swept = (int64_t)swept;
  for (int q = 0; q < nq; q++) {
    s.last_D += e->h_count[q];
    s.last_P += (int64_t)e->h_q_P[q];
    s.last_M += e->h_q_M[q];
    s.last_cand_pairs += e->h_pair_off[(size_t)q * (cn + 1) + cn];
  }
  stage_times(e);
  e->batch_synced = true;
  return SGTD_OK;
}

double est_matches_per_query(const sgtd_engine *e, int n_keypoints) {
  if (e->stats.last_queries > 0 && e->stats.last_D > 0 && e->nq > 0 && e->q_stride > 0) {
    const double per_slot = (double)e->stats.last_M / ((double)e->stats.last_queries * (double)e->q_stride);
    return per_slot * (double)n_keypoints * e->dc.tpi;
  }
  if (e->n_entries <= 0) return 0.0;
  const double L = (e->seg[0].sum_len_sq + (e->n_seg > 1 ? e->seg[1].sum_len_sq : 0.0)) / (double)e->n_entries;
  const double r = e->dc.rough / 0.03;
  const double per_desc = 0.55 * L * std::min(27.0, r * r * r) + 65.0;
  return 0.62 * (double)n_keypoints * e->dc.tpi * per_desc;
}

int settle_pending(sgtd_engine *e) {
  if (e->batch_valid && !e->batch_synced) return sync_batch(e);
  return SGTD_OK;
}

#define SGTD_TAIL_BATCHES 4
int settle_tail(sgtd_engine *e) {
  if (e->attached_to) return view_current(e);
  if (e->finalized && e->n_seg == 2) {
    if (e->tail_batches >= SGTD_TAIL_BATCHES) { e->tail_batches = 0; return do_finalize(e, true); }
    e->tail_batches++;
  } else {
    e->tail_batches = 1;
  }
  return do_finalize(e);
}

int remove_entries(sgtd_engine *e, const std::vector<u32> &bits, u32 span, int64_t *n_removed) {
  *n_removed = 0;
  const long long E = e->n_entries;
  const u32 lo = e->frame_lo, words = (u32)(((u64)span + 31) / 32);
  const long long n_tiles = (E + SGTD_RM_TILE - 1) / SGTD_RM_TILE;
  CHK(ensure(e, e->rm_bits, (size_t)words * sizeof(u32)));
  CHK(ensure(e, e->rm_present, (size_t)words * sizeof(u32)));
  CHK(ensure(e, e->rm_mask, (size_t)n_tiles * SGTD_RM_MASKS * sizeof(u64)));
  CHK(ensure(e, e->rm_count, (size_t)n_tiles * sizeof(u32)));
  HIPCHK(hipMemcpyAsync(e->rm_bits.p, bits.data(), (size_t)words * sizeof(u32), hipMemcpyHostToDevice, e->stream));
  HIPCHK(hipMemsetAsync(e->rm_present.p, 0, (size_t)words * sizeof(u32), e->stream));
  const int grid = (int)std::min<long long>(n_tiles, (long long)e->n_cus * 4);
  const size_t lds = (size_t)words * sizeof(u32);
  if (lds <= 65536) {
    remove_flag_kernel<true><<<grid, SGTD_RM_THREADS, lds, e->stream>>>(e->tab.frame.as<u32>(), E, e->rm_bits.as<u32>(), lo, span,
                                                                      e->rm_mask.as<u64>(), e->rm_count.as<u32>(), e->rm_present.as<u32>());
  } else {
    remove_flag_kernel<false><<<grid, SGTD_RM_THREADS, 0, e->stream>>>(e->tab.frame.as<u32>(), E, e->rm_bits.as<u32>(), lo, span,
                                                                     e->rm_mask.as<u64>(), e->rm_count.as<u32>(), e->rm_present.as<u32>());
  }
  HIPCHK(hipGetLastError());
  u32 last_cnt = 0, last_off = 0;
  std::vector<u32> present(words);
  HIPCHK(hipMemcpyAsync(&last_cnt, e->rm_count.as<u32>() + (n_tiles - 1), sizeof(u32), hipMemcpyDeviceToHost, e->stream));
  CHK(device_scan(e, e->rm_count.as<u32>(), e->rm_count.as<u32>(), n_tiles));
  HIPCHK(hipMemcpyAsync(&last_off, e->rm_count.as<u32>() + (n_tiles - 1), sizeof(u32), hipMemcpyDeviceToHost, e->stream));
  HIPCHK(hipMemcpyAsync(present.data(), e->rm_present.p, (size_t)words * sizeof(u32), hipMemcpyDeviceToHost, e->stream));
  HIPCHK(hipStreamSynchronize(e->stream));
  const long long kept = (long long)last_off + last_cnt;
  if (kept == E) {
    free_buf(e->rm_mask);
    free_buf(e->rm_count);
    return SGTD_OK;
  }
  if (kept > 0) {
    struct Field { DevBuf *buf; int w; };
    const Field fields[7] = {{&e->tab.vertex, 9}, {&e->tab.side, 6}, {&e->tab.angle, 6}, {&e->tab.center, 6},
                             {&e->tab.label, 3}, {&e->tab.node_id, 3}, {&e->tab.frame, 1}};
    for (const Field &f : fields) {
      CHK(ensure(e, e->rm_scratch, (size_t)kept * f.w * sizeof(u32)));
      const u32 *src = f.buf->as<u32>();
      u32 *dst = e->rm_scratch.as<u32>();
      const u64 *mask = e->rm_mask.as<u64>();
      const u32 *off = e->rm_count.as<u32>();
      const int tiles = (int)n_tiles;
      switch (f.w) {
        case 9: remove_compact_kernel<9><<<tiles, SGTD_RM_THREADS, 0, e->stream>>>(src, dst, E, mask, off); break;
        case 6: remove_compact_kernel<6><<<tiles, SGTD_RM_THREADS, 0, e->stream>>>(src, dst, E, mask, off); break;
        case 3: remove_compact_kernel<3><<<tiles, SGTD_RM_THREADS, 0, e->stream>>>(src, dst, E, mask, off); break;
        default: remove_compact_kernel<1><<<tiles, SGTD_RM_THREADS, 0, e->stream>>>(src, dst, E, mask, off); break;
      }
      HIPCHK(hipGetLastError());
      std::swap(*f.buf, e->rm_scratch);
      free_buf(e->rm_scratch);
    }
    size_t cap = SIZE_MAX;
    for (const Field &f : fields) cap = std::min(cap, f.buf->bytes / ((size_t)f.w * sizeof(u32)));
    e->tab.cap = cap;
  }
  long long gone_frames = 0;
  long long first = -1, last = -1;
  for (u32 w = 0; w < words; w++) {
    gone_frames += __builtin_popcount(present[w] & bits[w]);
    const u32 stay = present[w] & ~bits[w];
    if (stay) {
      if (first < 0) first = (long long)w * 32 + __builtin_ctz(stay);
      last = (long long)w * 32 + 31 - __builtin_clz(stay);
    }
  }
  free_buf(e->rm_mask);
  free_buf(e->rm_count);
  *n_removed = E - kept;
  e->n_entries = kept;
  e->n_add_calls = std::max<int64_t>(0, e->n_add_calls - gone_frames);
  e->have_frames = kept > 0;
  e->frame_lo = kept > 0 ? lo + (u32)first : 0;
  e->frame_hi = kept > 0 ? lo + (u32)last : 0;
  for (sgtd_engine::Segment &S : e->seg) { S.built = false; S.n_buckets = 0; S.sum_len_sq = 0.0; S.g0 = S.g1 = 0; }
  e->n_seg = 1;
  e->append_min_frame = 0xFFFFFFFFu;
  e->id_bits = 0;
  e->tail_batches = 0;
  e->finalized = false;
  e->batch_valid = false;
  e->table_version++;
  return SGTD_OK;
}

int check_cfg(const sgtd_config *c) {
  if (c->descriptor_near_num < 3 || c->descriptor_near_num > SGTD_MAX_K) return SGTD_ERR_UNSUPPORTED;
  if (c->candidate_num < 1 || c->candidate_num > SGTD_MAX_CAND) return SGTD_ERR_UNSUPPORTED;
  if (c->max_frame_n < 1) return SGTD_ERR_INVALID;
  if (!(c->std_side_resolution > 0) || !(c->descriptor_max_len > 0)) return SGTD_ERR_INVALID;
  if (!(c->descriptor_max_len * 1000.0 < 2097151.0)) return SGTD_ERR_UNSUPPORTED;
  if (!(c->descriptor_max_len / c->std_side_resolution + 2.0 < 65535.0)) return SGTD_ERR_UNSUPPORTED;
  return SGTD_OK;
}

}

namespace {
template <class T>
int stream_field(sgtd_engine *e, FILE *f, T *dev, size_t n_items, bool to_file, std::vector<char> &stage) {
  const size_t chunk = stage.size() / sizeof(T);
  for (size_t o = 0; o < n_items; o += chunk) {
    const size_t m = std::min(chunk, n_items - o);
    if (to_file) {
      HIPCHK(hipMemcpyAsync(stage.data(), dev + o, m * sizeof(T), hipMemcpyDeviceToHost, e->stream));
      HIPCHK(hipStreamSynchronize(e->stream));
      if (fwrite(stage.data(), sizeof(T), m, f) != m) return SGTD_ERR_IO;
    } else {
      if (fread(stage.data(), sizeof(T), m, f) != m) return SGTD_ERR_IO;
      HIPCHK(hipMemcpyAsync(dev + o, stage.data(), m * sizeof(T), hipMemcpyHostToDevice, e->stream));
      HIPCHK(hipStreamSynchronize(e->stream));
    }
  }
  return SGTD_OK;
}
int stream_table(sgtd_engine *e, FILE *f, size_t n, bool to_file) {
  std::vector<char> stage((size_t)64 << 20);
  CHK(stream_field(e, f, e->tab.side.as<double>(), n * 3, to_file, stage));
  CHK(stream_field(e, f, e->tab.angle.as<double>(), n * 3, to_file, stage));
  CHK(stream_field(e, f, e->tab.center.as<double>(), n * 3, to_file, stage));
  CHK(stream_field(e, f, e->tab.vertex.as<float>(), n * 9, to_file, stage));
  CHK(stream_field(e, f, e->tab.label.as<int>(), n * 3, to_file, stage));
  CHK(stream_field(e, f, e->tab.frame.as<u32>(), n, to_file, stage));
  CHK(stream_field(e, f, e->tab.node_id.as<int>(), n * 3, to_file, stage));
  return SGTD_OK;
}
}

extern "C" {

void sgtd_default_config(sgtd_config *cfg) {
  std::memset(cfg, 0, sizeof(*cfg));
  cfg->descriptor_near_num = 10;
  cfg->candidate_num = 50;
  cfg->max_frame_n = 20000;
  cfg->device_id = 0;
  cfg->descriptor_min_len = 0.5;
  cfg->descriptor_max_len = 50.0;
  cfg->std_side_resolution = 1.0;
  cfg->rough_dis_threshold = 0.03;
  cfg->first_frame_id = 0;
}

const char *sgtd_strerror(int status) {
  switch (status) {
    case SGTD_OK: return "ok";
    case SGTD_ERR_INVALID: return "invalid argument";
    case SGTD_ERR_NO_DEVICE: return "no usable gfx950 HIP device";
    case SGTD_ERR_HIP: return "HIP runtime error";
    case SGTD_ERR_CAPACITY: return "buffer capacity exceeded";
    case SGTD_ERR_FRAME_LIMIT: return "frame id beyond max_frame_n";
    case SGTD_ERR_UNSUPPORTED: return "configuration outside the kernels' envelope";
    case SGTD_ERR_STATE: return "call order";
    case SGTD_ERR_IO: return "graph file could not be opened or parsed";
    default: return "unknown status";
  }
}

const char *sgtd_last_error(sgtd_handle h) { return h ? h->err.c_str() : ""; }

uint32_t sgtd_label_code(int a, int b, int c) { return label_code(a, b, c); }
uint64_t sgtd_table_key(uint32_t code, uint32_t x, uint32_t y, uint32_t z) { return pack_key(code, x, y, z); }
uint64_t sgtd_dedup_key(uint64_t mx, uint64_t my, uint64_t mz) { return pack_milli_key(mx, my, mz); }

int sgtd_create(const sgtd_config *cfg, sgtd_handle *out) {
  if (!cfg || !out) return SGTD_ERR_INVALID;
  *out = nullptr;
  int r = check_cfg(cfg);
  if (r != SGTD_OK) return r;
  int ndev = 0;
  if (hipGetDeviceCount(&ndev) != hipSuccess || ndev <= 0) return SGTD_ERR_NO_DEVICE;
  if (cfg->device_id < 0 || cfg->device_id >= ndev) return SGTD_ERR_NO_DEVICE;
  hipDeviceProp_t prop;
  if (hipGetDeviceProperties(&prop, cfg->device_id) != hipSuccess) return SGTD_ERR_NO_DEVICE;
  if (std::strncmp(prop.gcnArchName, "gfx950", 6) != 0) return SGTD_ERR_NO_DEVICE;
  if (hipSetDevice(cfg->device_id) != hipSuccess) return SGTD_ERR_NO_DEVICE;
  sgtd_engine *e = new sgtd_engine();
  e->cfg = *cfg;
  e->dc.K = cfg->descriptor_near_num;
  e->dc.tpi = (cfg->descriptor_near_num - 1) * (cfg->descriptor_near_num - 2) / 2;
  e->dc.cand_num = cfg->candidate_num;
  e->dc.min_len = cfg->descriptor_min_len;
  e->dc.max_len = cfg->descriptor_max_len;
  e->dc.scale = 1.0 / cfg->std_side_resolution;
  e->dc.rough = cfg->rough_dis_threshold;
  e->n_cus = prop.multiProcessorCount > 0 ? prop.multiProcessorCount : 256;
  e->current_frame_id = cfg->first_frame_id;
  e->qd.with_thr2 = true;
  if (const char *o = getenv("SGTD_SORTED_CHUNK")) e->sorted_chunk = atoi(o);
  if (const char *o = getenv("SGTD_TAIL_MAX")) e->tail_max = atoll(o);
  if (const char *o = getenv("SGTD_COARSE_AT")) e->coarse_at = (u32)std::min(62ll, std::max(0ll, atoll(o)));
  if (const char *o = getenv("SGTD_REC_RATE")) e->rec_rate_hook = (u32)std::min(256, std::max(1, atoi(o)));
  if (const char *o = getenv("SGTD_WIDE_PAIRS")) e->wide_pairs = atoi(o) != 0;
  if (const char *o = getenv("SGTD_SELECT_MODE")) e->select_mode = std::min(2, std::max(0, atoi(o)));
  if (const char *o = getenv("SGTD_WHOLE_AT")) e->whole_at = (u32)std::min(62ll, std::max(0ll, atoll(o)));
  if (const char *o = getenv("SGTD_REC_CAP")) { e->rec_cap = (size_t)std::max(1024ll, atoll(o)); e->rec_cap_fixed = true; }
  if (const char *o = getenv("SGTD_POOL_UNITS")) e->pool_units = (size_t)std::max(64ll, atoll(o));
  if (const char *o = getenv("SGTD_GROUP_CAP")) e->group_cap_hook = (size_t)std::max(1ll, atoll(o));
  if (const char *o = getenv("SGTD_PAIR_CAP")) { e->pair_cap = (size_t)std::max(64ll, atoll(o)); e->rec_cap_fixed = true; }
  if (const char *o = getenv("SGTD_AMB_MIN")) e->amb_min = (size_t)std::max(1ll, atoll(o));
  for (int i = 0; i < EV_COUNT; i++)
    if (hipEventCreate(&e->ev[i]) != hipSuccess) { delete e; return SGTD_ERR_HIP; }
  if (hipEventCreateWithFlags(&e->ev_cand, hipEventDisableTiming) != hipSuccess ||
      hipEventCreateWithFlags(&e->ev_export_free, hipEventDisableTiming) != hipSuccess) { delete e; return SGTD_ERR_HIP; }
  *out = e;
  return SGTD_OK;
}

int sgtd_create_multi(const sgtd_config *cfg, const int *device_ids, int n_dev, sgtd_handle *out) {
  if (n_dev == 1 && cfg && device_ids && out) {
    sgtd_config c = *cfg;
    c.device_id = device_ids[0];
    return sgtd_create(&c, out);
  }
  return multi::create(cfg, device_ids, n_dev, out);
}

int sgtd_device_count(sgtd_handle e) { return !e ? 0 : (e->grp ? multi::device_count(e) : 1); }

sgtd_handle sgtd_device_handle(sgtd_handle e, int k) {
  if (!e) return nullptr;
  if (!e->grp) return k == 0 ? e : nullptr;
  return multi::device_handle(e, k);
}

int sgtd_destroy(sgtd_handle e) {
  if (e && e->grp) return multi::destroy(e);
  if (!e) return SGTD_OK;
  if (e->n_views > 0) { e->err = "other handles are attached to this handle's table (sgtd_attach_table): destroy them first"; return SGTD_ERR_STATE; }
  (void)hipSetDevice(e->cfg.device_id);
  (void)hipStreamSynchronize(e->stream);
  if (e->attached_to) { e->attached_to->n_views--; e->attached_to = nullptr; }
  free_store(e->tab); free_store(e->tmp); free_store(e->qd); free_store(e->fetch); free_buf(e->fetch_idx);
  DevBuf *bufs[] = {&e->seg[0].hot, &e->seg[0].perm, &e->seg[0].hash, &e->seg[0].bucket_start, &e->seg[0].bucket_key, &e->seg[0].dir,
                    &e->seg[1].hot, &e->seg[1].perm, &e->seg[1].hash, &e->seg[1].bucket_start, &e->seg[1].bucket_key, &e->seg[1].dir, &e->slice_of, &e->sq_sum,
                    &e->keyA, &e->keyB, &e->valA, &e->valB, &e->hist, &e->digit_tot, &e->flags, &e->bad_flag,
                    &e->kp_off_dev, &e->xyz_dev, &e->label_dev, &e->b_kp_off_dev, &e->b_xyz_dev, &e->b_label_dev, &e->ws_keys, &e->ws_slots, &e->cnt_scan,
                    &e->tmp_count, &e->q_count, &e->n_valid, &e->cell_rows, &e->gid, &e->q_prefix, &e->group_first, &e->n_groups, &e->pos_of_slot, &e->rec_off, &e->pass_pool, &e->v_score, &e->v_pose, &e->v_inlier, &e->v_best, &e->r_pose, &e->r_rmse, &e->r_rmse_v, &e->r_npairs, &e->r_moments, &e->r_flag, &e->kp_dev, &e->kp_word, &e->o_cnt, &e->o_val, &e->o_qxyz, &e->o_qlabel, &e->o_qoff, &e->a_pose, &e->a_fit, &e->a_cnt, &e->a_val, &e->a_mom, &e->a_assign, &e->inl_pairs, &e->inl_off, &e->v_hyp64, &e->v_hyp32, &e->v_bound, &e->v_hypB, &e->v_tau, &e->v_words, &e->v_okey[0], &e->v_okey[1], &e->v_oval[0], &e->v_oval[1], &e->cursors, &e->list, &e->n_visit,
                    &e->votes, &e->slot_of, &e->q_M, &e->q_P, &e->q_pairs, &e->q_pair_base,
                    &e->blk_count, &e->c_pair, &e->c_blk, &e->amb_queue, &e->rec, &e->rec_cell, &e->rec_dis, &e->rough_qi,
                    &e->rough_entry, &e->rough_frame, &e->rough_cell, &e->rough_dis, &e->n_cand, &e->cand_frame,
                    &e->cand_votes, &e->pair_off, &e->pairs, &e->totals, &e->inl_counts, &e->in_block, &e->b_in, &e->b_out,
                    &e->frame_first, &e->by_frame, &e->id_of_g, &e->longest,
                    &e->rm_bits, &e->rm_present, &e->rm_mask, &e->rm_count, &e->rm_scratch, &e->filt_rows,
                    &e->pos_dev, &e->prior_dev, &e->filt_base,
                    &e->ck_store, &e->ck_has, &e->ck_in, &e->ck_soa, &e->ck_valid, &e->ck_rows, &e->ck_pmask, &e->ck_out, &e->ck_state,
                    &e->cs_in, &e->cs_out,
                    &e->rx_in, &e->rx_state, &e->rx_edge, &e->rx_node, &e->rx_ctl};
  for (DevBuf *b : bufs) free_buf(*b);
  for (hipEvent_t ev : e->ck_ev)
    if (ev) (void)hipEventDestroy(ev);
  for (auto &b : e->scan_lvl) free_buf(b);
  if (e->pin) (void)hipHostFree(e->pin);
  if (e->frame_host) (void)hipHostFree(e->frame_host);
  if (e->pin_build) (void)hipHostFree(e->pin_build);
  for (int i = 0; i < EV_COUNT; i++)
    if (e->ev[i]) (void)hipEventDestroy(e->ev[i]);
  if (e->ev_cand) (void)hipEventDestroy(e->ev_cand);
  if (e->ev_export_free) (void)hipEventDestroy(e->ev_export_free);
  delete e;
  return SGTD_OK;
}

int sgtd_set_stream(sgtd_handle e, void *hip_stream) {
  if (e && e->grp) { e->err = "not available on a multi-device handle (use the per-device form, sgtd_amd/dist.py)"; return SGTD_ERR_UNSUPPORTED; }
  if (!e) return SGTD_ERR_INVALID;
  CHK(xfer_sync(e));
  e->stream = reinterpret_cast<hipStream_t>(hip_stream);
  return SGTD_OK;
}

int sgtd_set_timing(sgtd_handle e, int enabled) {
  if (e && e->grp) { for (int k = 0; k < sgtd_device_count(e); k++) sgtd_set_timing(sgtd_device_handle(e, k), enabled); return SGTD_OK; }
  if (!e) return SGTD_ERR_INVALID;
  e->timing = enabled != 0;
  return SGTD_OK;
}

int sgtd_current_frame_id(sgtd_handle e, uint32_t *out) {
  if (e && e->grp && out) { *out = multi::current_frame_id(e); return SGTD_OK; }
  if (!e || !out) return SGTD_ERR_INVALID;
  *out = e->current_frame_id;
  return SGTD_OK;
}

int64_t sgtd_max_descs(sgtd_handle e, int n_keypoints) {
  if (e && e->grp) return (int64_t)n_keypoints * ((e->cfg.descriptor_near_num - 1) * (e->cfg.descriptor_near_num - 2) / 2);
  if (!e || n_keypoints < 0) return 0;
  return (int64_t)n_keypoints * e->dc.tpi;
}

int sgtd_build(sgtd_handle e, const float *xyz, const uint32_t *label, int n, sgtd_desc_soa *out,
               int64_t capacity, int64_t *n_out) {
  PinScope pin_scope(e && !e->grp ? e : nullptr);
  if (e && e->grp) return multi::build(e, xyz, label, n, out, capacity, n_out);
  if (!e || !out || !n_out || n < 0 || (n > 0 && (!xyz || !label))) return SGTD_ERR_INVALID;
  HIPCHK(hipSetDevice(e->cfg.device_id));
  *n_out = 0;
  if (n == 0) return SGTD_OK;
  CHK(settle_pending(e));
  {
    const long long cap = (long long)n * e->dc.tpi;
    const size_t in_bytes = 16 + (size_t)n * 16, out_bytes = 16 + (size_t)cap * 136;
    if (out_bytes <= ((size_t)4 << 20) && n >= e->dc.K) {
#ifdef SGTD_EXP_FRAME_LAPS
      struct BLaps {
        std::chrono::steady_clock::time_point t0 = std::chrono::steady_clock::now(), t = t0;
        std::string s;
        void lap(const char *what) { const auto n = std::chrono::steady_clock::now(); char b[64]; snprintf(b, sizeof b, " %s %.0f", what, std::chrono::duration<double, std::micro>(n - t).count()); s += b; t = n; }
        ~BLaps() { fprintf(stderr, "[build laps us]%s | all %.0f\n", s.c_str(), std::chrono::duration<double, std::micro>(std::chrono::steady_clock::now() - t0).count()); }
      } blaps;
#define BLAP(x) blaps.lap(x)
#else
#define BLAP(x) do { } while (0)
#endif
      CHK(ensure(e, e->b_in, in_bytes));
      const size_t in_room = (in_bytes + 255) & ~(size_t)255;
      if (e->pin_build_cap < in_room + out_bytes) {
        if (e->pin_build) (void)hipHostFree(e->pin_build);
        e->pin_build = nullptr; e->pin_build_cap = 0;
        void *pp = nullptr;
        HIPCHK(hipHostMalloc(&pp, (in_room + out_bytes) * 2, hipHostMallocDefault));
        e->pin_build = static_cast<char *>(pp);
        e->pin_build_cap = (in_room + out_bytes) * 2;
      }
      char *hin = e->pin_build, *hout = e->pin_build + in_room;
      const long long off2[2] = {0, n};
      std::memcpy(hin, off2, 16);
      std::memcpy(hin + 16, xyz, (size_t)n * 12);
      std::memcpy(hin + 16 + (size_t)n * 12, label, (size_t)n * 4);
      HIPCHK(hipMemcpyAsync(e->b_in.p, hin, in_bytes, hipMemcpyHostToDevice, e->stream));
      BLAP("in");
      char *din = e->b_in.as<char>(), *dout = hout;
      DescArrays o;
      o.side = reinterpret_cast<double *>(dout + 16); o.angle = o.side + cap * 3; o.center = o.angle + cap * 3;
      o.vertex = reinterpret_cast<float *>(o.center + cap * 3); o.label = reinterpret_cast<int *>(o.vertex + cap * 9);
      o.frame = reinterpret_cast<u32 *>(o.label + cap * 3); o.node_id = reinterpret_cast<int *>(o.frame + cap);
      o.qrec = nullptr;
      CHK(launch_build(e, reinterpret_cast<const float *>(din + 16), reinterpret_cast<const u32 *>(din + 16 + (size_t)n * 12),
                       reinterpret_cast<const long long *>(din), 1, n, e->current_frame_id, 0, o, cap, reinterpret_cast<u32 *>(dout)));
      BLAP("launch");
      HIPCHK(hipStreamSynchronize(e->stream));
      BLAP("out_and_wait");
      const u32 cnt = *reinterpret_cast<const u32 *>(hout);
      *n_out = cnt;
      if ((int64_t)cnt > capacity) return SGTD_ERR_CAPACITY;
      const char *hp = hout + 16;
      auto take = [&](void *dst, size_t width, size_t elem) {
        if (dst) std::memcpy(dst, hp, (size_t)cnt * width * elem);
        hp += (size_t)cap * width * elem;
      };
      take(out->side, 3, 8); take(out->angle, 3, 8); take(out->center, 3, 8); take(out->vertex, 9, 4); take(out->label, 3, 4);
      take(out->frame, 1, 4); take(out->node_id, 3, 4);
      BLAP("fields");
#undef BLAP
      return SGTD_OK;
    }
  }
  int64_t off[2] = {0, n};
  const float *dx; const u32 *dl; int max_n;
  CHK(stage_inputs(e, xyz, label, off, 1, 0, &dx, &dl, &max_n, true));
  const long long stride = (long long)n * e->dc.tpi;
  CHK(ensure_store(e, e->tmp, (size_t)std::max<long long>(stride, 1)));
  CHK(ensure(e, e->tmp_count, sizeof(u32)));
  CHK(launch_build(e, dx, dl, e->b_kp_off_dev.as<long long>(), 1, max_n, e->current_frame_id, 0,
                   e->tmp.view(), stride, e->tmp_count.as<u32>()));
  u32 cnt = 0;
  CHK(d2h(e, &cnt, e->tmp_count.p, sizeof(u32)));
  CHK(xfer_sync(e));
  *n_out = cnt;
  if ((int64_t)cnt > capacity) return SGTD_ERR_CAPACITY;
  return copy_out(e, e->tmp, 0, cnt, out, 0);
}

int sgtd_add(sgtd_handle e, const sgtd_desc_soa *d, int64_t n) {
  if (e && e->grp) return multi::add(e, d, n);
  if (!e || n < 0 || (n > 0 && (!d || !d->side || !d->label || !d->frame))) return SGTD_ERR_INVALID;
  HIPCHK(hipSetDevice(e->cfg.device_id));
  u32 lo = 0xFFFFFFFFu, hi = 0;
  for (int64_t i = 0; i < n; i++) {
    lo = std::min(lo, d->frame[i]);
    hi = std::max(hi, d->frame[i]);
  }
  if (n > 0 && hi >= (u32)e->cfg.max_frame_n) return SGTD_ERR_FRAME_LIMIT;
  if (e->attached_to) { e->err = "the table belongs to another handle (sgtd_attach_table): add to its owner"; return SGTD_ERR_STATE; }
  CHK(settle_pending(e));
  e->table_version++;
  e->current_frame_id++;
  e->n_add_calls++;
// ... 2403 lines not shown
```

Baseline: 191,300.

## Add fused one-sweep radix sort with decoupled lookback for home-cell ordering

Adds a fused ordering path for the per-query home-cell sort. Key generation now builds all four digit histograms in one kernel. Each radix pass is a single one-sweep kernel that uses decoupled lookback across tiles, and group detection uses a lookback scan as well. This replaces the multi-kernel sort and scan sequence and its extra launches and memsets. The lookback spins under a poll budget with a give-up flag; when it trips, the batch falls back to the old path via a rerun, which adds complexity and a possible deadlock-avoidance cost.

```diff
diff --git a/include/sgtd_accel.h b/include/sgtd_accel.h
--- a/include/sgtd_accel.h
+++ b/include/sgtd_accel.h
@@ -70,8 +70,10 @@
   int64_t device_allocs_total;
   float ms_consistency_pairs, ms_consistency_greedy;
   int32_t consistency_rounds;
-  int32_t reserved3;
+  int32_t order_giveups_total;
 } sgtd_stats;
+
+void sgtd_order_tiles(int *sort_tile, int *group_tile);
 
 typedef struct sgtd_engine *sgtd_handle;
 
diff --git a/sgtd_amd/_lib.py b/sgtd_amd/_lib.py
--- a/sgtd_amd/_lib.py
+++ b/sgtd_amd/_lib.py
@@ -16,7 +16,7 @@
     "sgtd_add", "sgtd_add_frames", "sgtd_finalize", "sgtd_query_frames", "sgtd_query_descs", "sgtd_max_batch",
     "sgtd_result_candidates", "sgtd_export_candidates_dev", "sgtd_result_query_desc_count", "sgtd_result_pairs",
     "sgtd_result_query_descs", "sgtd_result_votes", "sgtd_result_rough", "sgtd_fetch_entries", "sgtd_host_alloc", "sgtd_host_free",
-    "sgtd_table_dump", "sgtd_sync", "sgtd_get_stats",
+    "sgtd_table_dump", "sgtd_sync", "sgtd_get_stats", "sgtd_order_tiles",
     "sgtd_verify", "sgtd_export_verify_dev", "sgtd_result_verify", "sgtd_result_inliers", "sgtd_result_inlier_pairs", "sgtd_result_inlier_entries", "sgtd_search_loop",
     "sgtd_graphs_load", "sgtd_graphs_save_cache", "sgtd_graphs_load_cache", "sgtd_graphs_view",
     "sgtd_graphs_error", "sgtd_graphs_free", "sgtd_save_table", "sgtd_load_table",
@@ -81,7 +81,7 @@
         ("tail_entries", C.c_int64), ("ms_finalize", C.c_float), ("reserved2", C.c_float),
         ("batches_total", C.c_int64), ("overflow_launches_total", C.c_int64), ("reruns_total", C.c_int64), ("rewrites_total", C.c_int64),
         ("list_moves_total", C.c_int64), ("last_list_moves", C.c_int64), ("device_allocs_total", C.c_int64),
-        ("ms_consistency_pairs", C.c_float), ("ms_consistency_greedy", C.c_float), ("consistency_rounds", C.c_int32), ("reserved3", C.c_int32),
+        ("ms_consistency_pairs", C.c_float), ("ms_consistency_greedy", C.c_float), ("consistency_rounds", C.c_int32), ("order_giveups_total", C.c_int32),
     ]
 
 
@@ -195,6 +195,8 @@
     L.sgtd_sync.argtypes = [vp]
     L.sgtd_max_batch.argtypes = [vp, C.c_int, C.POINTER(C.c_int64)]
     L.sgtd_get_stats.argtypes = [vp, C.POINTER(Stats)]
+    L.sgtd_order_tiles.argtypes = [C.POINTER(C.c_int), C.POINTER(C.c_int)]
+    L.sgtd_order_tiles.restype = None
     L.sgtd_verify.argtypes = [vp]
     L.sgtd_result_verify.argtypes = [vp, C.c_int, vp, vp]
     L.sgtd_export_verify_dev.argtypes = [vp, vp, vp]
diff --git a/sgtd_amd/csrc/multi_impl.hip.h b/sgtd_amd/csrc/multi_impl.hip.h
--- a/sgtd_amd/csrc/multi_impl.hip.h
+++ b/sgtd_amd/csrc/multi_impl.hip.h
@@ -679,7 +679,7 @@
     t.overflowed |= x.overflowed;
     t.select_form = x.select_form;
     t.batches_total = x.batches_total; t.overflow_launches_total += x.overflow_launches_total;
-    t.reruns_total += x.reruns_total; t.rewrites_total += x.rewrites_total;
+    t.reruns_total += x.reruns_total; t.rewrites_total += x.rewrites_total; t.order_giveups_total += x.order_giveups_total;
     t.list_moves_total += x.list_moves_total; t.last_list_moves += x.last_list_moves;
     t.ms_total = std::max(t.ms_total, x.ms_total);
     if (s == 0) { t.ms_consistency_pairs = x.ms_consistency_pairs; t.ms_consistency_greedy = x.ms_consistency_greedy; t.consistency_rounds = x.consistency_rounds; }
diff --git a/sgtd_amd/csrc/order_kernels.hip.h b/sgtd_amd/csrc/order_kernels.hip.h
--- /dev/null
+++ b/sgtd_amd/csrc/order_kernels.hip.h
@@ -0,0 +1,317 @@
+#pragma once
+#include "probe_kernels.hip.h"
+
+#define SGTD_OS_THREADS 512
+#define SGTD_OS_ITEMS 16
+#define SGTD_OS_TILE (SGTD_OS_THREADS * SGTD_OS_ITEMS)
+#define SGTD_GI_THREADS 256
+#define SGTD_GI_ITEMS 16
+#define SGTD_GI_TILE (SGTD_GI_THREADS * SGTD_GI_ITEMS)
+#define SGTD_ORDER_WINDOW 8
+#define SGTD_ORDER_POLLS_DEFAULT (1u << 20)
+#define SGTD_ORDER_MAX_KEYS (1ll << 30)
+
+enum { OW_TICKET = 0, OW_GROUP_TICKET = 4, OW_HIST = 64, OW_STATE = OW_HIST + 4 * 256 };
+__host__ __device__ __forceinline__ size_t order_sort_state_at(int pass, u32 tiles_cap) { return (size_t)OW_STATE + (size_t)pass * tiles_cap * 256; }
+__host__ __device__ __forceinline__ size_t order_group_state_at(int passes, u32 tiles_cap) { return (order_sort_state_at(passes, tiles_cap) + 1) & ~(size_t)1; }
+__host__ __device__ __forceinline__ size_t order_work_words(int passes, u32 tiles_cap, u32 gtiles_cap) { return order_group_state_at(passes, tiles_cap) + (size_t)gtiles_cap * 2; }
+
+#define SGTD_ST_AGG 1u
+#define SGTD_ST_INCL 2u
+#define SGTD_ST_MASK 0x3FFFFFFFu
+
+__device__ __forceinline__ u32 order_ld(const u32 *p) { return __hip_atomic_load(p, __ATOMIC_RELAXED, __HIP_MEMORY_SCOPE_AGENT); }
+__device__ __forceinline__ void order_st(u32 *p, u32 v) { __hip_atomic_store(p, v, __ATOMIC_RELAXED, __HIP_MEMORY_SCOPE_AGENT); }
+__device__ __forceinline__ u64 order_ld64(const u64 *p) { return __hip_atomic_load(p, __ATOMIC_RELAXED, __HIP_MEMORY_SCOPE_AGENT); }
+__device__ __forceinline__ void order_st64(u64 *p, u64 v) { __hip_atomic_store(p, v, __ATOMIC_RELAXED, __HIP_MEMORY_SCOPE_AGENT); }
+
+__global__ __launch_bounds__(256) void order_begin_kernel(const u32 *count, u32 *q_prefix, int n_queries, u32 *n_valid, u32 *q_M, unsigned long long *q_P) {
+  __shared__ u32 lds[256 / SGTD_WAVE + 1];
+  for (int q = threadIdx.x; q < n_queries; q += 256) { q_M[q] = 0u; q_P[q] = 0ull; }
+  u32 carry = 0;
+  for (int q0 = 0; q0 < n_queries; q0 += 256) {
+    const int q = q0 + threadIdx.x;
+    const u32 v = (q < n_queries) ? count[q] : 0;
+    u32 tot;
+    const u32 ex = block_excl_scan(v, lds, tot);
+    if (q < n_queries) q_prefix[q] = carry + ex;
+    carry += tot;
+  }
+  if (threadIdx.x == 0) *n_valid = carry;
+}
+
+__global__ __launch_bounds__(256) void home_keys_hist_kernel(QueryView Q, const u32 *q_prefix, u32 *keys, u32 *vals, long long n_slots, int cbits, int sub_bits,
+                                                             u32 *hist, u32 *pos_of_slot, size_t n_pass_slots) {
+  __shared__ u32 h[4 * 256];
+  for (int i = threadIdx.x; i < 4 * 256; i += 256) h[i] = 0u;
+  __syncthreads();
+  const u64 cmask = (1ull << cbits) - 1ull;
+  const int ny = 1 << (sub_bits >> 1), nz = 1 << (sub_bits - (sub_bits >> 1));
+  for (long long d = (long long)blockIdx.x * 256 + threadIdx.x; d < n_slots; d += (long long)gridDim.x * 256) {
+    const int q = (int)(d / Q.stride);
+    const u32 i = (u32)(d - (long long)q * Q.stride);
+    if (i >= Q.count[q]) continue;
+    const u64 code = label_code(Q.label[d * 3 + 0], Q.label[d * 3 + 1], Q.label[d * 3 + 2]);
+    const double s0 = Q.side[d * 3 + 0], s1 = Q.side[d * 3 + 1], s2 = Q.side[d * 3 + 2];
+    const u64 x = home_coord(s0, cmask), y = home_coord(s1, cmask), z = home_coord(s2, cmask);
+    const double f1 = s1 - (double)(int)s1, f2 = s2 - (double)(int)s2;
+    const u64 sub = (u64)min(max((int)(f1 * ny), 0), ny - 1) * nz + (u64)min(max((int)(f2 * nz), 0), nz - 1);
+    const u32 key = (u32)(((((code << cbits | x) << cbits | y) << cbits) | z) << sub_bits | sub);
+    const u32 idx = q_prefix[q] + i;
+    keys[idx] = key;
+    vals[idx] = (u32)d;
+#pragma unroll
+    for (int b = 0; b < 4; b++) atomicAdd(&h[b * 256 + ((key >> (8 * b)) & 255u)], 1u);
+  }
+  __syncthreads();
+  for (int i = threadIdx.x; i < 4 * 256; i += 256)
+    if (h[i]) atomicAdd(&hist[i], h[i]);
+  uint4 *p4 = reinterpret_cast<uint4 *>(pos_of_slot);
+  const size_t n4 = n_pass_slots / 4, step = (size_t)gridDim.x * 256, first = (size_t)blockIdx.x * 256 + threadIdx.x;
+  for (size_t i = first; i < n4; i += step) p4[i] = make_uint4(SGTD_NO_PASS, SGTD_NO_PASS, SGTD_NO_PASS, SGTD_NO_PASS);
+  for (size_t i = n4 * 4 + first; i < n_pass_slots; i += step) pos_of_slot[i] = SGTD_NO_PASS;
+}
+
+__global__ __launch_bounds__(SGTD_OS_THREADS) __attribute__((amdgpu_waves_per_eu(4))) void order_sort_pass_kernel(
+const u32 *keys_in, const u32 *vals_in, u32 *keys_out, u32 *vals_out,
+                                                                          const u32 *n_valid_p, long long n_cap, u32 *work, u32 tiles_cap, int pass,
+                                                                          u32 max_polls, u32 *giveup) {
+  constexpr int NW = SGTD_OS_THREADS / SGTD_WAVE;
+  constexpr u32 PER_WAVE = SGTD_OS_TILE / NW;
+  __shared__ u32 s_key[SGTD_OS_TILE], s_val[SGTD_OS_TILE];
+  __shared__ u32 s_wcnt[NW][256];
+  __shared__ u32 s_start[256];
+  __shared__ u32 s_gbase[256];
+  __shared__ u32 s_scan[NW + 1];
+  __shared__ u32 s_tile, s_quit;
+  const u32 tid = threadIdx.x, wid = tid >> 6, lane = tid & 63u;
+  const u32 nv = (u32)min((long long)*n_valid_p, n_cap);
+  const u32 ntiles = min((nv + SGTD_OS_TILE - 1u) / SGTD_OS_TILE, tiles_cap);
+  if (blockIdx.x >= ntiles) return;
+  if (tid == 0) { s_tile = atomicAdd(&work[OW_TICKET + pass], 1u); s_quit = order_ld(giveup); }
+  for (u32 i = tid; i < NW * 256u; i += SGTD_OS_THREADS) (&s_wcnt[0][0])[i] = 0u;
+  __syncthreads();
+  const u32 tile = s_tile;
+  if (s_quit || tile >= ntiles) return;
+  u32 *state = work + order_sort_state_at(pass, tiles_cap);
+  const u32 base = tile * SGTD_OS_TILE, n_tile = min((u32)SGTD_OS_TILE, nv - base);
+  const int shift = 8 * pass;
+  u32 key[SGTD_OS_ITEMS], place[SGTD_OS_ITEMS];
+#pragma unroll
+  for (int r = 0; r < SGTD_OS_ITEMS; r++) {
+    const u32 i = wid * PER_WAVE + (u32)r * SGTD_WAVE + lane;
+    key[r] = i < n_tile ? keys_in[base + i] : 0xFFFFFFFFu;
+  }
+#pragma unroll
+  for (int r = 0; r < SGTD_OS_ITEMS; r++) {
+    const u32 i = wid * PER_WAVE + (u32)r * SGTD_WAVE + lane;
+    const bool valid = i < n_tile;
+    const u32 digit = (key[r] >> shift) & 255u;
+    u32 rank, count;
+    wave_group_rank<8>(digit, valid, rank, count);
+    const u32 have = s_wcnt[wid][digit];
+    __builtin_amdgcn_wave_barrier();
+    if (valid && rank == 0) s_wcnt[wid][digit] = have + count;
+    __builtin_amdgcn_wave_barrier();
+    place[r] = have + rank;
+  }
+  __syncthreads();
+  u32 cnt = 0;
+  if (tid < 256u) {
+#pragma unroll
+    for (int w = 0; w < NW; w++) { const u32 t = s_wcnt[w][tid]; s_wcnt[w][tid] = cnt; cnt += t; }
+    order_st(&state[(size_t)tile * 256 + tid], ((tile == 0 ? SGTD_ST_INCL : SGTD_ST_AGG) << 30) | cnt);
+  }
+  u32 tot;
+  const u32 start = block_excl_scan(cnt, s_scan, tot);
+  const u32 gstart = block_excl_scan(tid < 256u ? work[OW_HIST + pass * 256 + tid] : 0u, s_scan, tot);
+  u32 before = 0;
+  bool quit = false;
+  if (tid < 256u && tile > 0) {
+    u32 polls = max_polls, idle = 0, t = tile;
+    bool done = false;
+    while (!done) {
+      if (polls == 0) { quit = true; break; }
+      polls -= min(polls, (u32)SGTD_ORDER_WINDOW);
+      u32 s[SGTD_ORDER_WINDOW];
+#pragma unroll
+      for (int w = 0; w < SGTD_ORDER_WINDOW; w++) s[w] = (u32)w < t ? order_ld(&state[(size_t)(t - 1u - (u32)w) * 256 + tid]) : 0u;
+      const u32 t0 = t;
+      bool stop = false;
+#pragma unroll
+      for (int w = 0; w < SGTD_ORDER_WINDOW; w++) {
+        if (stop || (u32)w >= t0) continue;
+        if ((s[w] >> 30) == 0u) { stop = true; continue; }
+        before += s[w] & SGTD_ST_MASK;
+        t = t0 - 1u - (u32)w;
+        if ((s[w] >> 30) == SGTD_ST_INCL || t == 0u) { done = true; stop = true; }
+      }
+      if (t == t0) {
+        if ((++idle & 255u) == 0u && order_ld(giveup)) { quit = true; break; }
+        __builtin_amdgcn_s_sleep(2);
+      }
+    }
+    if (quit) { order_st(giveup, 1u); s_quit = 1u; }
+    else order_st(&state[(size_t)tile * 256 + tid], (SGTD_ST_INCL << 30) | (before + cnt));
+  }
+  if (tid < 256u) { s_start[tid] = start; s_gbase[tid] = gstart + before - start; }
+  __syncthreads();
+  if (s_quit) return;
+  u32 val[SGTD_OS_ITEMS];
+#pragma unroll
+  for (int r = 0; r < SGTD_OS_ITEMS; r++) {
+    const u32 i = wid * PER_WAVE + (u32)r * SGTD_WAVE + lane;
+    val[r] = i < n_tile ? vals_in[base + i] : 0u;
+  }
+#pragma unroll
+  for (int r = 0; r < SGTD_OS_ITEMS; r++) {
+    const u32 i = wid * PER_WAVE + (u32)r * SGTD_WAVE + lane;
+    if (i < n_tile) {
+      const u32 digit = (key[r] >> shift) & 255u;
+      const u32 at = s_start[digit] + s_wcnt[wid][digit] + place[r];
+      s_key[at] = key[r];
+      s_val[at] = val[r];
+    }
+  }
+  __syncthreads();
+  for (u32 j = tid; j < n_tile; j += SGTD_OS_THREADS) {
+    const u32 k = s_key[j];
+    const u32 g = s_gbase[(k >> shift) & 255u] + j;
+    if (g < nv) { keys_out[g] = k; vals_out[g] = s_val[j]; }
+  }
+}
+
+__device__ __forceinline__ u32 wave_incl_max_scan(u32 v) {
+  int x = (int)v;
+#define SGTD_MAX_STEP(ctrl, rows) { const u32 o = (u32)__builtin_amdgcn_update_dpp(0, x, ctrl, rows, 0xf, false); x = (int)((u32)x > o ? (u32)x : o); }
+  SGTD_MAX_STEP(0x111, 0xf) SGTD_MAX_STEP(0x112, 0xf) SGTD_MAX_STEP(0x114, 0xf) SGTD_MAX_STEP(0x118, 0xf)
+  SGTD_MAX_STEP(0x142, 0xa) SGTD_MAX_STEP(0x143, 0xc)
+#undef SGTD_MAX_STEP
+  return (u32)x;
+}
+
+__device__ __forceinline__ bool order_group_head(u32 key, u32 key_before, int cbits, int sub_bits) {
+  const u32 a = key >> sub_bits, b = key_before >> sub_bits;
+  const u32 cmask = (1u << cbits) - 1u;
+  return (a != b) || ((a & cmask) == cmask) || (((a >> cbits) & cmask) == cmask) || (((a >> (2 * cbits)) & cmask) == cmask);
+}
+
+__global__ __launch_bounds__(SGTD_GI_THREADS) void order_groups_kernel(const u32 *keys, u32 *n_valid_p, u32 *gid, u32 *group_first, u32 *n_groups,
+                                                                       u32 *pos_of_slot, u32 slot_cap, long long n_cap, u32 *ticket, u64 *state,
+                                                                       u32 tiles_cap, int cbits, int sub_bits, int pair, u32 max_polls, u32 *giveup,
+                                                                       int *overflow) {
+  constexpr int NW = SGTD_GI_THREADS / SGTD_WAVE;
+  __shared__ u32 s_scan[NW + 1], s_max[NW];
+  __shared__ u32 s_tile, s_quit, s_heads, s_last;
+  const u32 tid = threadIdx.x, wid = tid >> 6, lane = tid & 63u;
+  const u32 nv = (u32)min((long long)*n_valid_p, n_cap);
+  if (order_ld(giveup)) {
+    if (blockIdx.x == 0 && tid == 0) { order_st(n_valid_p, 0u); order_st(n_groups, 0u); order_st(reinterpret_cast<u32 *>(overflow), 1u); }
+    return;
+  }
+  if (nv == 0) { if (blockIdx.x == 0 && tid == 0) *n_groups = 0u; return; }
+  const u32 ntiles = min((nv + SGTD_GI_TILE - 1u) / SGTD_GI_TILE, tiles_cap);
+  if (blockIdx.x >= ntiles) return;
+  if (tid == 0) { s_tile = atomicAdd(ticket, 1u); s_quit = 0u; }
+  __syncthreads();
+  const u32 tile = s_tile;
+  if (tile >= ntiles) return;
+  const u32 p0 = tile * SGTD_GI_TILE + tid * SGTD_GI_ITEMS;
+  const bool full = (tile + 1u) * SGTD_GI_TILE <= nv;
+  u32 k[SGTD_GI_ITEMS];
+  if (full) {
+    const uint4 *src = reinterpret_cast<const uint4 *>(keys + p0);
+#pragma unroll
+    for (int j = 0; j < SGTD_GI_ITEMS / 4; j++) { const uint4 w = src[j]; k[4 * j] = w.x; k[4 * j + 1] = w.y; k[4 * j + 2] = w.z; k[4 * j + 3] = w.w; }
+  } else {
+#pragma unroll
+    for (int j = 0; j < SGTD_GI_ITEMS; j++) k[j] = p0 + j < nv ? keys[p0 + j] : 0u;
+  }
+  u32 before = (p0 > 0 && p0 < nv) ? keys[p0 - 1] : 0u;
+  u32 heads = 0, mine = 0, last = 0;
+#pragma unroll
+  for (int j = 0; j < SGTD_GI_ITEMS; j++) {
+    const u32 p = p0 + j;
+    const bool h = p < nv && (p == 0 || order_group_head(k[j], before, cbits, sub_bits));
+    before = k[j];
+    if (h) { heads |= 1u << j; mine++; last = p + 1u; }
+  }
+  u32 tile_heads;
+  const u32 ex_heads = block_excl_scan(mine, s_scan, tile_heads);
+  const u32 inc_last = wave_incl_max_scan(last);
+  if (lane == SGTD_WAVE - 1) s_max[wid] = inc_last;
+  __syncthreads();
+  u32 ex_last = (u32)__shfl_up((int)inc_last, 1);
+  if (lane == 0) ex_last = 0;
+  u32 tile_last = 0;
+#pragma unroll
+  for (int w = 0; w < NW; w++) { const u32 m = s_max[w]; if ((u32)w < wid) ex_last = max(ex_last, m); tile_last = max(tile_last, m); }
+  if (tid == 0) {
+    u32 c_heads = 0, c_last = 0;
+    bool quit = false;
+    if (tile > 0) {
+      order_st64(&state[tile], ((u64)SGTD_ST_AGG << 62) | ((u64)tile_heads << 31) | (u64)tile_last);
+      u32 polls = max_polls, idle = 0, t = tile;
+      bool done = false;
+      while (!done) {
+        if (polls == 0) { quit = true; break; }
+        polls -= min(polls, (u32)SGTD_ORDER_WINDOW);
+        u64 s[SGTD_ORDER_WINDOW];
+#pragma unroll
+        for (int w = 0; w < SGTD_ORDER_WINDOW; w++) s[w] = (u32)w < t ? order_ld64(&state[t - 1u - (u32)w]) : 0ull;
+        const u32 t0 = t;
+        bool stop = false;
+#pragma unroll
+        for (int w = 0; w < SGTD_ORDER_WINDOW; w++) {
+          if (stop || (u32)w >= t0) continue;
+          if ((s[w] >> 62) == 0ull) { stop = true; continue; }
+          c_heads += (u32)(s[w] >> 31) & 0x7FFFFFFFu;
+          if (c_last == 0) c_last = (u32)s[w] & 0x7FFFFFFFu;
+          t = t0 - 1u - (u32)w;
+          if ((u32)(s[w] >> 62) == SGTD_ST_INCL || t == 0u) { done = true; stop = true; }
+        }
+        if (t == t0) {
+          if ((++idle & 255u) == 0u && order_ld(giveup)) { quit = true; break; }
+          __builtin_amdgcn_s_sleep(2);
+        }
+      }
+    }
+    if (quit) {
+      order_st(giveup, 1u); order_st(n_valid_p, 0u); order_st(n_groups, 0u); order_st(reinterpret_cast<u32 *>(overflow), 1u);
+      s_quit = 1u;
+    } else {
+      order_st64(&state[tile], ((u64)SGTD_ST_INCL << 62) | ((u64)(c_heads + tile_heads) << 31) | (u64)(tile_last ? tile_last : c_last));
+    }
+    s_heads = c_heads; s_last = c_last;
+  }
+  __syncthreads();
+  if (s_quit) return;
+  u32 H = s_heads + ex_heads, F = ex_last ? ex_last : s_last;
+  u32 g[SGTD_GI_ITEMS];
+#pragma unroll
+  for (int j = 0; j < SGTD_GI_ITEMS; j++) {
+    const u32 p = p0 + j;
+    if ((heads >> j) & 1u) { H++; F = p + 1u; }
+    g[j] = H - 1u;
+    if (p < nv) {
+      if (((heads >> j) & 1u) && H <= nv) group_first[H - 1u] = p;
+      if (!pair) pos_of_slot[p] = p;
+      else {
+        const u32 f = F - 1u;
+        if (((p - f) % SGTD_PAIR) == 0u) {
+          const u32 s = (H - 1u) + (f + SGTD_PAIR - 1u) / SGTD_PAIR + (p - f) / SGTD_PAIR;
+          if (s < slot_cap) pos_of_slot[s] = p;
+        }
+      }
+      if (p == nv - 1u) *n_groups = H;
+    }
+  }
+  if (full) {
+    uint4 *dst = reinterpret_cast<uint4 *>(gid + p0);
+#pragma unroll
+    for (int j = 0; j < SGTD_GI_ITEMS / 4; j++) dst[j] = make_uint4(g[4 * j], g[4 * j + 1], g[4 * j + 2], g[4 * j + 3]);
+  } else {
+#pragma unroll
+    for (int j = 0; j < SGTD_GI_ITEMS; j++) if (p0 + j < nv) gid[p0 + j] = g[j];
+  }
+}
diff --git a/sgtd_amd/csrc/probe_kernels.hip.h b/sgtd_amd/csrc/probe_kernels.hip.h
--- a/sgtd_amd/csrc/probe_kernels.hip.h
+++ b/sgtd_amd/csrc/probe_kernels.hip.h
@@ -35,7 +35,7 @@
 
 #define SGTD_REC_SHIFT 2
 enum { CTR_REC_CURSOR = 0, CTR_AMB_COUNT = 2, CTR_COMPACT_CURSOR = 3, CTR_REC_NEED = 4, CTR_SWEPT = 6, CTR_POOL_CURSOR = 8, CTR_LIST_MOVES = 9,
-       CTR_OVERFLOW = 10, CTR_COUNT = 12, CTR_XCD_HEADS = 1024 };
+       CTR_OVERFLOW = 10, CTR_COUNT = 12, CTR_ORDER_GIVEUP = 16, CTR_XCD_HEADS = 1024 };
 struct ProbeBuffers {
   u32 *rec;
   unsigned char *rec_cell;
diff --git a/sgtd_amd/csrc/sgtd_accel.hip b/sgtd_amd/csrc/sgtd_accel.hip
--- a/sgtd_amd/csrc/sgtd_accel.hip
+++ b/sgtd_amd/csrc/sgtd_accel.hip
@@ -17,6 +17,7 @@
 #include "common.hip.h"
 #include "table_kernels.hip.h"
 #include "probe_kernels.hip.h"
+#include "order_kernels.hip.h"
 #include "select_kernels.hip.h"
 #include "verify_kernels.hip.h"
 #include "verify_mfma.hip.h"
@@ -114,6 +115,7 @@
   u32 tile_span = 1, n_tiles = 1; size_t hist_bytes = 0; bool lds_votes = false;
   bool votes_fit = false, table_fits = false, per_query = false, fused_pairs = false, fused_votes = false, votes_per_query = false;
   int cbits = 1, sub_bits = 0, key_bits = 0; bool small = false, pair = false; size_t max_pass_slots = 0;
+  bool order_fused = false; u32 order_tiles = 0, order_gtiles = 0;
   int row_slots = 1; u32 ticket = 2; int sgrid = 0, pgrid = 0; bool narrow = false, frames = false;
   bool narrow_pairs = false;
 };
@@ -192,6 +194,7 @@
   } prior_key;
   bool prior_rows_valid = false;
   DevBuf keyA, keyB, valA, valB, hist, digit_tot, flags, bad_flag;
+  DevBuf order_work;
   std::vector<DevBuf> scan_lvl;
 
   DevBuf kp_off_dev, xyz_dev, label_dev, ws_keys, ws_slots, cnt_scan;
@@ -288,6 +291,10 @@
   size_t amb_min = 65536;
   int sorted_chunk = 0;
   bool diag = false;
+  int order_form = -1;
+  u32 order_polls = SGTD_ORDER_POLLS_DEFAULT;
+  bool order_gave_up = false;
+  bool order_train = false;
   int select_mode = 0;
   PinnedVec<u32> h_count, h_pair_base, h_q_M;
   PinnedVec<unsigned long long> h_q_P;
@@ -922,6 +929,11 @@
   p.key_bits = 12 + 3 * p.cbits + p.sub_bits;
   const bool small_on = [] { const char *o = getenv("SGTD_SMALL_ORDER"); return !(o && !atoi(o)); }();
   p.small = small_on && nq == 1 && n_slots <= SGTD_SMALL_SLOTS && p.key_bits <= 32 && !p.fused_votes && span <= (1u << 20);
+  const bool small_shape = nq == 1 && n_slots <= SGTD_SMALL_SLOTS;
+  p.order_fused = !p.small && (e->order_form == 1 || (e->order_form < 0 && !small_shape)) && !e->order_train && p.key_bits <= 32 && n_slots > 0 &&
+                  n_slots < SGTD_ORDER_MAX_KEYS;
+  p.order_tiles = (u32)((n_slots + SGTD_OS_TILE - 1) / SGTD_OS_TILE);
+  p.order_gtiles = (u32)((n_slots + SGTD_GI_TILE - 1) / SGTD_GI_TILE);
   p.pair = !e->diag && SGTD_PAIR >= 2;
   p.max_pass_slots = (size_t)pass_slot_count((u32)n_slots, (u32)n_slots, p.pair) + 64;
   p.row_slots = e->n_seg > 1 ? 2 : 1;
@@ -1186,6 +1198,7 @@
   for (DevBuf *b : {&e->valA, &e->valB, &e->gid, &e->group_first}) CHK(ensure(e, *b, n_slots * sizeof(u32)));
   for (DevBuf *b : {&e->n_valid, &e->n_groups}) CHK(ensure(e, *b, sizeof(u32)));
   for (DevBuf *b : {&e->pos_of_slot, &e->rec_off}) CHK(ensure(e, *b, p.max_pass_slots * sizeof(u32)));
+  if (p.order_fused) CHK(ensure(e, e->order_work, order_work_words((p.key_bits + 7) / 8, p.order_tiles, p.order_gtiles) * sizeof(u32)));
   if (e->pool_units == 0) e->pool_units = std::max<size_t>(65536, n_slots * (e->n_entries > 100000000 ? 16 : 10));
   CHK(ensure(e, e->pass_pool, (e->pool_units + SGTD_PASS_SLACK_UNITS) * sizeof(uint4)));
   return SGTD_OK;
@@ -1206,8 +1219,36 @@
     HIPCHK(hipMemsetAsync(e->cand_frame.p, 0xFF, (size_t)nq * cn * sizeof(int), e->stream));
     HIPCHK(hipMemsetAsync(e->cand_votes.p, 0, (size_t)nq * cn * sizeof(int), e->stream));
   }
+  if (p.order_fused) return SGTD_OK;
   HIPCHK(hipMemsetAsync(e->q_M.p, 0, (size_t)nq * sizeof(u32), e->stream));
   HIPCHK(hipMemsetAsync(e->q_P.p, 0, (size_t)nq * sizeof(unsigned long long), e->stream));
+  return SGTD_OK;
+}
+
+int order_fused(sgtd_engine *e, const SelectPlan &p, const Views &v, u32 **order) {
+  const long long n_slots = p.n_slots;
+  const int passes = (p.key_bits + 7) / 8;
+  u32 *kin = e->keyA.as<u32>(), *kout = e->keyB.as<u32>(), *vin = e->valA.as<u32>(), *vout = e->valB.as<u32>();
+  u32 *nv = e->n_valid.as<u32>(), *work = e->order_work.as<u32>(), *giveup = e->cursors.as<u32>() + CTR_ORDER_GIVEUP;
+  order_begin_kernel<<<1, 256, 0, e->stream>>>(e->q_count.as<u32>(), e->q_prefix.as<u32>(), p.nq, nv, e->q_M.as<u32>(),
+                                               e->q_P.as<unsigned long long>());
+  HIPCHK(hipGetLastError());
+  HIPCHK(hipMemsetAsync(work, 0, order_work_words(passes, p.order_tiles, p.order_gtiles) * sizeof(u32), e->stream));
+  home_keys_hist_kernel<<<(unsigned)std::min<long long>(grid_for(n_slots, 256), (long long)e->n_cus * 8), 256, 0, e->stream>>>(v.Q, e->q_prefix.as<u32>(), kin, vin, n_slots,
+                                                                                                                              p.cbits, p.sub_bits, work + OW_HIST, e->pos_of_slot.as<u32>(), p.max_pass_slots);
+  HIPCHK(hipGetLastError());
+  for (int pass = 0; pass < passes; pass++) {
+    order_sort_pass_kernel<<<p.order_tiles, SGTD_OS_THREADS, 0, e->stream>>>(kin, vin, kout, vout, nv, n_slots, work, p.order_tiles, pass, e->order_polls, giveup);
+    HIPCHK(hipGetLastError());
+    std::swap(kin, kout);
+    std::swap(vin, vout);
+  }
+  order_groups_kernel<<<p.order_gtiles, SGTD_GI_THREADS, 0, e->stream>>>(kin, nv, e->gid.as<u32>(), e->group_first.as<u32>(), e->n_groups.as<u32>(), e->pos_of_slot.as<u32>(),
+                                                                        (u32)std::min<size_t>(p.max_pass_slots, 0xFFFFFFFFu), n_slots, work + OW_GROUP_TICKET,
+                                                                        reinterpret_cast<u64 *>(work + order_group_state_at(passes, p.order_tiles)), p.order_gtiles, p.cbits,
+                                                                        p.sub_bits, p.pair ? 1 : 0, e->order_polls, giveup, v.B.overflow());
+  HIPCHK(hipGetLastError());
+  e->thr2_pending = 0; *order = vin;
   return SGTD_OK;
 }
 
@@ -1232,6 +1273,7 @@
     e->thr2_pending = 0; *order = vin;
     return SGTD_OK;
   }
+  if (p.order_fused) return order_fused(e, p, v, order);
   query_prefix_kernel<<<1, 256, 0, e->stream>>>(e->q_count.as<u32>(), e->q_prefix.as<u32>(), p.nq, e->n_valid.as<u32>());
   HIPCHK(hipGetLastError());
   auto sort_by_home = [&](auto *kin, auto *kout) -> int {
@@ -1432,9 +1474,13 @@
 }
 
 int rerun(sgtd_engine *e) {
-  if (e->last_kind == 1) return enqueue_frames(e);
-  if (e->timing) HIPCHK(hipEventRecord(e->ev[EV_START], e->stream));
-  return launch_select(e);
+  e->order_train = e->order_gave_up;
+  int st = SGTD_OK;
+  if (e->last_kind == 1) st = enqueue_frames(e);
+  else if (e->timing && hipEventRecord(e->ev[EV_START], e->stream) != hipSuccess) st = SGTD_ERR_HIP;
+  else st = launch_select(e);
+  e->order_train = false;
+  return st;
 }
 
 int rerun_write(sgtd_engine *e) {
@@ -1476,6 +1522,7 @@
   CHK(view_current(e));
   if (e->batch_synced) return SGTD_OK;
   e->stats.overflowed = 0;
+  e->order_gave_up = false;
   unsigned long long swept = 0;
   for (int attempt = 0; attempt < 12; attempt++) {
     int ovf[2] = {0, 0};
@@ -1507,6 +1554,17 @@
       fprintf(stderr, "sgtd: batch re-run (attempt %d): flags %d %d, records %llu of %zu (+%llu wanted), pass pool %u of %zu units, home cells %u of %zu rows, pairs %u of %zu\n",
               attempt, ovf[0], ovf[1], cursor, e->rec_cap, need, pool_used, e->pool_units, n_groups, e->group_cap, total, e->pair_cap);
     if (attempt == 11) return SGTD_ERR_CAPACITY;
+    if (ovf[0] && e->plan.order_fused) {
+      u32 gave_up = 0;
+      CHK(d2h(e, &gave_up, e->cursors.as<u32>() + CTR_ORDER_GIVEUP, sizeof(u32)));
+      CHK(xfer_sync(e));
+      if (gave_up) {
+        e->stats.order_giveups_total++;
+        e->order_gave_up = true;
+        CHK(rerun(e));
+        continue;
+      }
+    }
     const size_t lim = kRecLimit, pair_lim = kIndexLimit;
     if (ovf[0] && (size_t)n_groups > e->group_cap) {
       e->group_cap = (size_t)n_groups + (size_t)n_groups / 4 + 1024;
@@ -1723,6 +1781,11 @@
 }
 
 extern "C" {
+
+void sgtd_order_tiles(int *sort_tile, int *group_tile) {
+  if (sort_tile) *sort_tile = SGTD_OS_TILE;
+  if (group_tile) *group_tile = SGTD_GI_TILE;
+}
 
 void sgtd_default_config(sgtd_config *cfg) {
   std::memset(cfg, 0, sizeof(*cfg));
@@ -1787,6 +1850,8 @@
   if (const char *o = getenv("SGTD_COARSE_AT")) e->coarse_at = (u32)std::min(62ll, std::max(0ll, atoll(o)));
   if (const char *o = getenv("SGTD_REC_RATE")) e->rec_rate_hook = (u32)std::min(256, std::max(1, atoi(o)));
   if (const char *o = getenv("SGTD_WIDE_PAIRS")) e->wide_pairs = atoi(o) != 0;
+  if (const char *o = getenv("SGTD_ORDER_FORM")) e->order_form = atoi(o) != 0 ? 1 : 0;
+  if (const char *o = getenv("SGTD_ORDER_POLLS")) e->order_polls = (u32)std::min(1ll << 30, std::max(0ll, atoll(o)));
   if (const char *o = getenv("SGTD_SELECT_MODE")) e->select_mode = std::min(2, std::max(0, atoi(o)));
   if (const char *o = getenv("SGTD_WHOLE_AT")) e->whole_at = (u32)std::min(62ll, std::max(0ll, atoll(o)));
   if (const char *o = getenv("SGTD_REC_CAP")) { e->rec_cap = (size_t)std::max(1024ll, atoll(o)); e->rec_cap_fixed = true; }
@@ -1829,7 +1894,7 @@
   free_store(e->tab); free_store(e->tmp); free_store(e->qd); free_store(e->fetch); free_buf(e->fetch_idx);
   DevBuf *bufs[] = {&e->seg[0].hot, &e->seg[0].perm, &e->seg[0].hash, &e->seg[0].bucket_start, &e->seg[0].bucket_key, &e->seg[0].dir,
                     &e->seg[1].hot, &e->seg[1].perm, &e->seg[1].hash, &e->seg[1].bucket_start, &e->seg[1].bucket_key, &e->seg[1].dir, &e->slice_of, &e->sq_sum,
-                    &e->keyA, &e->keyB, &e->valA, &e->valB, &e->hist, &e->digit_tot, &e->flags, &e->bad_flag,
+                    &e->keyA, &e->keyB, &e->valA, &e->valB, &e->hist, &e->digit_tot, &e->flags, &e->bad_flag, &e->order_work,
                     &e->kp_off_dev, &e->xyz_dev, &e->label_dev, &e->b_kp_off_dev, &e->b_xyz_dev, &e->b_label_dev, &e->ws_keys, &e->ws_slots, &e->cnt_scan,
                     &e->tmp_count, &e->q_count, &e->n_valid, &e->cell_rows, &e->gid, &e->q_prefix, &e->group_first, &e->n_groups, &e->pos_of_slot, &e->rec_off, &e->pass_pool, &e->v_score, &e->v_pose, &e->v_inlier, &e->v_best, &e->r_pose, &e->r_rmse, &e->r_rmse_v, &e->r_npairs, &e->r_moments, &e->r_flag, &e->kp_dev, &e->kp_word, &e->o_cnt, &e->o_val, &e->o_qxyz, &e->o_qlabel, &e->o_qoff, &e->a_pose, &e->a_fit, &e->a_cnt, &e->a_val, &e->a_mom, &e->a_assign, &e->inl_pairs, &e->inl_off, &e->v_hyp64, &e->v_hyp32, &e->v_bound, &e->v_hypB, &e->v_tau, &e->v_words, &e->v_okey[0], &e->v_okey[1], &e->v_oval[0], &e->v_oval[1], &e->cursors, &e->list, &e->n_visit,
                     &e->votes, &e->slot_of, &e->q_M, &e->q_P, &e->q_pairs, &e->q_pair_base,
```

Result: faster. 196,800, median of 6 (+2.9%).
